# shamim-hussain/egt

Measured on AMD Instinct MI355X. Metric: graphs/sec EGT fwd+bwd, ZINC-500K padded N=64, higher is better.
Workload: dtype f32; 1 GPU; zinc500k_n64: attention-block stack (h,e,mask)->(h',e') x Ly, fwd+bwd + param grads; scope=stack, graphs_per_gpu=128, global_batch=128, N=64, Dh=64, De=64, H=8, d=8, Ly=10, parallelism=dp1, grad_allreduce_bytes=740480, backend=none (single process), flat_grad_adopted=True, flat_grad_bound=True, collective_in_graph=False

## Files before the change

### egt_amd/_lib.py

```python
from __future__ import annotations

import ctypes as C
import os

_HERE = os.path.dirname(os.path.abspath(__file__))
LIB_PATH = os.environ.get("EGT_AMD_LIB") or os.path.join(_HERE, "lib", "libegt_amd.so")

ABI_VERSION = 4
EGT_OK = 0
EGT_E_NULL, EGT_E_SHAPE, EGT_E_DTYPE, EGT_E_FLAGS, EGT_E_HIP, EGT_E_WORKSPACE, EGT_E_RCCL = -1, -2, -3, -4, -5, -6, -7
EGT_F32 = 0
EGT_BF16 = 1
F_EDGE_INPUT, F_GATE_INPUT, F_ATTN_MASK, F_SCALE_DEGREE = 0x001, 0x002, 0x004, 0x008
F_SCALER_LINEAR, F_TRAINING, F_CLIP = 0x010, 0x020, 0x040
ATTN_WS_SHARED = 0x1
EP_LAYERNORM, EP_GATES = 0x1, 0x2
ACT_NONE, ACT_LRELU, ACT_RELU, ACT_ELU = 0, 1, 2, 3
BF_GATE, BF_ATTN_MASK, BF_TRAINING, BF_CLIP, BF_NO_EDGE_LN, BF_SEED_DEVICE = 0x1, 0x2, 0x4, 0x8, 0x10, 0x20
BF_STATIC_EDGE = 0x40


class AttnDesc(C.Structure):
    _fields_ = [("B", C.c_int32), ("N", C.c_int32), ("H", C.c_int32), ("d", C.c_int32),
                ("dtype", C.c_int32), ("flags", C.c_uint32),
                ("clip_lo", C.c_float), ("clip_hi", C.c_float),
                ("random_mask_prob", C.c_float), ("attn_dropout", C.c_float),
                ("num_virtual_nodes", C.c_int32), ("reserved", C.c_int32),
                ("seed", C.c_uint64)]


class EdgeDesc(C.Structure):
    _fields_ = [("rows", C.c_int64), ("De", C.c_int32), ("H", C.c_int32),
                ("dtype", C.c_int32), ("flags", C.c_uint32), ("act", C.c_int32),
                ("act_alpha", C.c_float), ("ln_eps", C.c_float), ("reserved", C.c_int32)]


class BlockDesc(C.Structure):
    _fields_ = [("B", C.c_int32), ("N", C.c_int32), ("H", C.c_int32), ("d", C.c_int32),
                ("De", C.c_int32), ("dtype", C.c_int32), ("flags", C.c_uint32),
                ("clip_lo", C.c_float), ("clip_hi", C.c_float),
                ("random_mask_prob", C.c_float), ("ln_eps", C.c_float),
                ("reserved", C.c_int32), ("seed", C.c_uint64), ("seed_device", C.c_void_p)]


class FfnDesc(C.Structure):
    _fields_ = [("rows", C.c_int64), ("width", C.c_int32), ("dtype", C.c_int32),
                ("activation", C.c_int32), ("ln_eps", C.c_float), ("matmul", C.c_int32), ("flags", C.c_int32)]


MM_F32, MM_BF16X3, MM_BF16 = 0, 1, 2
FFN_WS_PREPARED = 1


FFN_PARAM_FIELDS = ("norm_gamma", "norm_beta", "lr1_kernel", "lr1_bias", "lr2_kernel", "lr2_bias")


class FfnParams(C.Structure):
    _fields_ = [(n, C.c_void_p) for n in FFN_PARAM_FIELDS]


BLOCK_PARAM_FIELDS = (
    "norm_edge_gamma", "norm_edge_beta",
    "attention_gates_kernel", "attention_gates_bias",
    "dense_edge_b_kernel", "dense_edge_b_bias",
    "norm_mha_gamma", "norm_mha_beta",
    "dense_qkv_kernel", "dense_qkv_bias",
    "dense_mha_kernel", "dense_mha_bias",
    "dense_edge_r_kernel", "dense_edge_r_bias",
)


class BlockParams(C.Structure):
    _fields_ = [(n, C.c_void_p) for n in BLOCK_PARAM_FIELDS]


class EmbedDesc(C.Structure):
    _fields_ = [("B", C.c_int32), ("N", C.c_int32), ("De", C.c_int32), ("upto_hop", C.c_int32),
                ("clip_hops", C.c_int32), ("num_edge_features", C.c_int32), ("dtype", C.c_int32),
                ("num_float_features", C.c_int32), ("mask_value", C.c_float), ("reserved", C.c_int32)]


EH_LAYERNORM = 0x1


class HeadDesc(C.Structure):
    _fields_ = [("B", C.c_int32), ("N", C.c_int32), ("De", C.c_int32), ("M0", C.c_int32), ("M1", C.c_int32),
                ("C", C.c_int32), ("dtype", C.c_int32), ("activation", C.c_int32), ("flags", C.c_int32),
                ("ln_eps", C.c_float), ("reserved", C.c_int32)]


HEAD_PARAM_FIELDS = ("edge_norm_final_gamma", "edge_norm_final_beta", "mlp_out_dist_targ_0_kernel",
                     "mlp_out_dist_targ_0_bias", "mlp_out_dist_targ_1_kernel", "mlp_out_dist_targ_1_bias",
                     "distance_target_kernel", "distance_target_bias")


class HeadParams(C.Structure):
    _fields_ = [(n, C.c_void_p) for n in HEAD_PARAM_FIELDS]


class EGTLibraryError(RuntimeError):
    pass


_lib = None

_VP = C.c_void_p
_PROTOS = {
    "egt_last_error_string": (C.c_char_p, []),
    "egt_abi_version": (C.c_int, []),
    "egt_attn_fwd": (C.c_int, [C.POINTER(AttnDesc)] + [_VP] * 12),
    "egt_attn_bwd_workspace_bytes": (C.c_size_t, [C.POINTER(AttnDesc)]),
    "egt_attn_bwd": (C.c_int, [C.POINTER(AttnDesc)] + [_VP] * 16),
    "egt_attn_mfma_supported": (C.c_int, [C.POINTER(AttnDesc), C.c_int]),
    "egt_attn_mfma_fwd_workspace_bytes": (C.c_size_t, [C.POINTER(AttnDesc)]),
    "egt_attn_mfma_workspace_bytes": (C.c_size_t, [C.POINTER(AttnDesc)]),
    "egt_attn_mfma_fwd": (C.c_int, [C.POINTER(AttnDesc)] + [_VP] * 11),
    "egt_attn_mfma_bwd": (C.c_int, [C.POINTER(AttnDesc)] + [_VP] * 15),
    "egt_mask_sample": (C.c_int, [C.c_int, C.c_uint64, C.c_float, C.c_int32, C.c_int32,
                                  C.c_int32, _VP, _VP]),
    "egt_seed_advance": (C.c_int, [_VP, C.c_int32, C.c_uint64, _VP]),
    "egt_edge_proj_fwd": (C.c_int, [C.POINTER(EdgeDesc)] + [_VP] * 10),
    "egt_edge_proj_bwd_workspace_bytes": (C.c_size_t, [C.POINTER(EdgeDesc)]),
    "egt_edge_proj_bwd": (C.c_int, [C.POINTER(EdgeDesc)] + [_VP] * 17),
    "egt_edge_proj_bwd_acc": (C.c_int, [C.POINTER(EdgeDesc)] + [_VP] * 18),
    "egt_edge_update_fwd": (C.c_int, [C.POINTER(EdgeDesc)] + [_VP] * 6),
    "egt_edge_update_bwd_workspace_bytes": (C.c_size_t, [C.POINTER(EdgeDesc)]),
    "egt_edge_update_bwd": (C.c_int, [C.POINTER(EdgeDesc)] + [_VP] * 8),
    "egt_node_mask_from_features": (C.c_int, [_VP, C.c_int32, C.c_int32, C.c_int32, _VP, _VP]),
    "egt_node_mask_from_float_features": (C.c_int, [_VP, C.c_int32, C.c_int32, C.c_int32, C.c_float, C.c_int32, _VP, _VP]),
    "egt_constrained_edge_mask": (C.c_int, [_VP, C.c_int32, C.c_int32, C.c_int32, C.c_int32, _VP, _VP]),
    "egt_edge_embed_supported": (C.c_int, [C.POINTER(EmbedDesc)]),
    "egt_edge_embed_hops_bytes": (C.c_size_t, [C.POINTER(EmbedDesc)]),
    "egt_edge_embed_workspace_bytes": (C.c_size_t, [C.POINTER(EmbedDesc)]),
    "egt_edge_embed_fwd": (C.c_int, [C.POINTER(EmbedDesc)] + [_VP] * 9),
    "egt_edge_embed_bwd": (C.c_int, [C.POINTER(EmbedDesc)] + [_VP] * 8),
    "egt_distance_target": (C.c_int, [_VP, C.c_int32, C.c_int32, C.c_int32, _VP, _VP]),
    "egt_edge_head_supported": (C.c_int, [C.POINTER(HeadDesc)]),
    "egt_edge_head_workspace_bytes": (C.c_size_t, [C.POINTER(HeadDesc)]),
    "egt_edge_head_fwd": (C.c_int, [C.POINTER(HeadDesc), C.POINTER(HeadParams)] + [_VP] * 5),
    "egt_edge_head_bwd": (C.c_int, [C.POINTER(HeadDesc), C.POINTER(HeadParams)] + [_VP] * 4
                          + [C.POINTER(HeadParams)] + [_VP] * 2),
    "egt_dp_unique_id": (C.c_int, [_VP]),
    "egt_dp_init": (C.c_int, [_VP, C.c_int32, C.c_int32]),
    "egt_dp_allreduce": (C.c_int, [_VP, C.c_size_t, C.c_int32, _VP]),
    "egt_dp_world": (C.c_int, []),
    "egt_dp_rank": (C.c_int, []),
    "egt_dp_finalize": (C.c_int, []),
    "egt_prof_enable": (C.c_int, [C.c_int]),
    "egt_prof_filter": (C.c_int, [C.c_char_p]),
    "egt_prof_stride": (C.c_int, [C.c_int]),
    "egt_prof_read": (C.c_int, [C.c_char_p, C.POINTER(C.c_int64), C.POINTER(C.c_double)]),
    "egt_prof_names": (C.c_int, [C.c_char_p, C.c_size_t]),
    "egt_prof_collect_graph": (C.c_int, [C.c_int]),
    "egt_prof_forget_graphs": (C.c_int, []),
    "egt_block_supported": (C.c_int, [C.POINTER(BlockDesc)]),
    "egt_block_bwd_kernel": (C.c_char_p, [C.POINTER(BlockDesc)]),
    "egt_block_launch_form": (C.c_char_p, [C.POINTER(BlockDesc)]),
    "egt_block_saved_bytes": (C.c_size_t, [C.POINTER(BlockDesc)]),
    "egt_block_workspace_bytes": (C.c_size_t, [C.POINTER(BlockDesc)]),
    "egt_block_fwd": (C.c_int, [C.POINTER(BlockDesc), C.POINTER(BlockParams)] + [_VP] * 10),
    "egt_block_bwd": (C.c_int, [C.POINTER(BlockDesc), C.POINTER(BlockParams)] + [_VP] * 10
                      + [C.POINTER(BlockParams)] + [_VP] * 2),
    "egt_stack_saved_bytes": (C.c_size_t, [C.POINTER(BlockDesc), C.c_int32]),
    "egt_stack_workspace_bytes": (C.c_size_t, [C.POINTER(BlockDesc), C.c_int32]),
    "egt_stack_fwd": (C.c_int, [C.POINTER(BlockDesc), C.c_int32, C.POINTER(BlockParams)] + [_VP] * 9),
    "egt_stack_bwd": (C.c_int, [C.POINTER(BlockDesc), C.c_int32, C.POINTER(BlockParams)] + [_VP] * 9
                      + [C.POINTER(BlockParams)] + [_VP] * 2),
    "egt_pair_supported": (C.c_int, [C.POINTER(BlockDesc)]),
    "egt_pair_workspace_bytes": (C.c_size_t, [C.POINTER(BlockDesc)]),
    "egt_pair_fwd": (C.c_int, [C.POINTER(BlockDesc), C.POINTER(BlockParams)] + [_VP] * 8),
    "egt_pair_bwd": (C.c_int, [C.POINTER(BlockDesc), C.POINTER(BlockParams)] + [_VP] * 9
                     + [C.POINTER(BlockParams)] + [_VP] * 2),
    "egt_ffn_supported": (C.c_int, [C.POINTER(FfnDesc)]),
    "egt_ffn_workspace_bytes": (C.c_size_t, [C.POINTER(FfnDesc)]),
    "egt_ffn_fwd": (C.c_int, [C.POINTER(FfnDesc), C.POINTER(FfnParams)] + [_VP] * 4),
    "egt_ffn_bwd": (C.c_int, [C.POINTER(FfnDesc), C.POINTER(FfnParams)] + [_VP] * 3
                    + [C.POINTER(FfnParams)] + [_VP] * 2),
}


def load():
    global _lib
    if _lib is not None:
        return _lib
    if not os.path.exists(LIB_PATH):
        raise EGTLibraryError(
            f"{LIB_PATH} not found: build the HIP extension first "
            "(python -c 'import __graft_entry__ as g; g.build()' or python egt_amd/build.py)")
    lib = C.CDLL(LIB_PATH)
    for name, (res, args) in _PROTOS.items():
        fn = getattr(lib, name)
        fn.restype, fn.argtypes = res, args
    if lib.egt_abi_version() != ABI_VERSION:
        raise EGTLibraryError("ABI version mismatch")
    _lib = lib
    return lib


_EXC = {EGT_E_NULL: ValueError, EGT_E_SHAPE: AssertionError, EGT_E_DTYPE: TypeError,
        EGT_E_FLAGS: ValueError, EGT_E_HIP: RuntimeError, EGT_E_WORKSPACE: RuntimeError, EGT_E_RCCL: RuntimeError}


def check(rc: int):
    if rc == EGT_OK:
        return
    msg = load().egt_last_error_string().decode(errors="replace")
    raise _EXC.get(rc, RuntimeError)(f"egt_amd: {msg} (code {rc})")


def ptr(t):
    return None if t is None else C.c_void_p(t.data_ptr())


def current_stream():
    import torch
    return C.c_void_p(torch.cuda.current_stream().cuda_stream)
```

### egt_amd/csrc/egt_block.hip

```cpp
#include "egt_common.h"

#include <stdio.h>
#include <stdlib.h>
#include <string.h>
#include <vector>

#include "egt_block.h"
#include "egt_tile.h"

#include "egt_block_dev.h"
#include "egt_dma.h"

#include "egt_block_fwd.h"
#include "egt_block_bwd.h"



struct EgtBlockEnv {
  bool no_narrow_fwd, no_narrow_bwd;
  int bwd_mm;
  int bwd_tl, fwd_rows;
  int nrw_fwd_waves, nrw_bwd_waves, nrw_fwd_half;
};
static bool env_flag_raw(const char* name) {
  const char* v = getenv(name);
  return v && v[0] && v[0] != '0';
}
static int env_int(const char* name, int unset) {
  const char* v = getenv(name);
  return v ? atoi(v) : unset;
}
static const EgtBlockEnv& block_env() {
  static const EgtBlockEnv e = [] {
    EgtBlockEnv v{};
    v.no_narrow_fwd = env_flag_raw("EGT_NO_NARROW_FWD") || env_flag_raw("EGT_NO_NARROW");
    v.no_narrow_bwd = env_flag_raw("EGT_NO_NARROW_BWD") || env_flag_raw("EGT_NO_NARROW");
    const char* mm = getenv("EGT_BWD_MATMUL");
    v.bwd_mm = (mm && !strcmp(mm, "bf16x3")) ? EGT_MM_BF16X3 : EGT_MM_F32;
    v.bwd_tl = env_int("EGT_BWD_TL", 0);
    v.fwd_rows = env_int("EGT_FWD_ROWS", 0);
    v.nrw_fwd_waves = env_int("EGT_NRW_FWD_WAVES", 0);
    v.nrw_bwd_waves = env_int("EGT_NRW_BWD_WAVES", 0);
    v.nrw_fwd_half = env_int("EGT_NRW_FWD_HALF", -1);
    return v;
  }();
  return e;
}
int egt_device_cus() {
  static const int n = [] {
    int dev = 0, cu = 256;
    if (hipGetDevice(&dev) == hipSuccess) (void)hipDeviceGetAttribute(&cu, hipDeviceAttributeMultiprocessorCount, dev);
    return cu > 0 ? cu : 256;
  }();
  return n;
}

static int block_check(const egt_block_desc* d, bool report) {
#define BAD(code, ...) do { if (report) egt_set_error(__VA_ARGS__); return (code); } while (0)
  if (!d) BAD(EGT_E_NULL, "desc is NULL");
  if (d->dtype != EGT_F32 && d->dtype != EGT_BF16) BAD(EGT_E_DTYPE, "dtype must be EGT_F32 or EGT_BF16 (got %d)", d->dtype);
  if (d->B <= 0 || d->N <= 0) BAD(EGT_E_SHAPE, "B and N must be positive");
  if (d->H != BH) BAD(EGT_E_SHAPE, "fused block is built for num_heads=8 (got %d)", d->H);
  if (d->d < 1 || d->d > 8) BAD(EGT_E_SHAPE, "fused block covers per-head dim <= 8 (got %d)", d->d);
  switch (d->De) {
    case 8: case 16: case 32: case 48: case 64: break;
    default: BAD(EGT_E_SHAPE, "fused block covers edge_width in {8,16,32,48,64} (got %d)", d->De);
  }
  if ((size_t)d->B * d->N * d->N * d->H > 0xFFFFFFFFull) BAD(EGT_E_SHAPE, "B*N*N*H exceeds the 32-bit RNG counter");
  if ((d->flags & EGT_BF_SEED_DEVICE) && !d->seed_device) BAD(EGT_E_NULL, "EGT_BF_SEED_DEVICE set but seed_device is NULL");
  if (d->flags & EGT_BF_STATIC_EDGE) {
    if (!(d->flags & EGT_BF_NO_EDGE_LN)) BAD(EGT_E_FLAGS, "EGT_BF_STATIC_EDGE is only valid together with EGT_BF_NO_EDGE_LN");
    if (d->flags & EGT_BF_ATTN_MASK) BAD(EGT_E_FLAGS, "EGT_BF_STATIC_EDGE does not take EGT_BF_ATTN_MASK");
    if (d->De != 8) BAD(EGT_E_SHAPE, "EGT_BF_STATIC_EDGE covers edge_width 8 (got %d)", d->De);
    if (block_env().no_narrow_fwd || block_env().no_narrow_bwd) BAD(EGT_E_FLAGS, "EGT_BF_STATIC_EDGE needs the De = 8 pair kernels (EGT_NO_NARROW* is set)");
  }
  return EGT_OK;
#undef BAD
}

extern "C" int egt_block_supported(const egt_block_desc* d) { return block_check(d, false) == EGT_OK; }

static size_t al(size_t x) { return (x + 63) & ~(size_t)63; }

enum class FwdKernel { narrow, r4, tile };
enum class BwdKernel { narrow, v4r, v5, v4 };
static const char* const g_bwd_kernel_name[] = {"k_narrow_bwd", "k_block_bwd_v4r", "k_block_bwd_v5", "k_block_bwd_v4"};
constexpr int V4R_RR = 2;

struct BlockPlan {
  bool ml;
  bool full;
  FwdKernel fwd;
  EgtLaunch fl;
  int fwd_nw;
  bool fwd_half;
  bool kvl;
  bool epi_ok;
  int RGF;
  BwdKernel bwd;
  EgtLaunch bl;
  int bwd_nw;
  int mm;
  int TL, NLR, nwg_bwd, EP;
  size_t v_att, stats, qkvp, pw_sv, wfrag_sv, saved_total;
  size_t dvp, dqp, dkvp, dqp_sz, dkvp_sz, common_total;
  size_t pw, epart, spart, sbo, wpart, ered, dqkv, dhbuf, layer_total;
};

template <int DE>
static BlockPlan plan_for(const egt_block_desc* d, bool ml) {
  using GG = Geo<DE>;
  const EgtBlockEnv& E = block_env();
  const int B = d->B, N = d->N, cus = egt_device_cus();
  const int groups = (N + BWD_TL - 1) / BWD_TL;
  BlockPlan P{};
  P.ml = ml;
  P.full = (N % 16) == 0;

  int tg = 2 * cus / B;
  {
    const int cap = B * ((N + 3) / 4) <= cus ? (N + 3) / 4 : (N + 7) / 8;
    if (tg > cap) tg = cap;
  }

  P.RGF = tg > groups ? (((N + tg - 1) / tg + 3) / 4) * 4 : 16;
  if (E.fwd_rows >= 4 && E.fwd_rows <= 16) P.RGF = E.fwd_rows;
  const size_t lds_tiles = (size_t)8 * GG::TILE_FLOATS * 4;
  const size_t lds_kv = ((size_t)N * KV_LD + 16 * QS_LD + N) * 4;
  P.kvl = lds_tiles + lds_kv <= 80 * 1024 - 512;
  const size_t lds_r4 = (size_t)16 * GG::TILE_FLOATS * 4 + lds_kv;
  const size_t lds_r8 = (size_t)32 * GG::TILE_FLOATS * 4 + ((size_t)N * KV_LD + 32 * QS_LD + N) * 4;
  const bool r4 = lds_r4 <= 80 * 1024 - 512, r8 = !r4 && lds_r8 <= 156 * 1024;
  if (DE == 8 && !ml && !E.no_narrow_fwd) {
    const int grid16 = B * groups;
    P.fwd = FwdKernel::narrow;
    P.fwd_nw = E.nrw_fwd_waves == 8 || (E.nrw_fwd_waves != 4 && grid16 <= cus && N >= 64) ? 8 : 4;
    P.fwd_half = P.fwd_nw == 8 && (E.nrw_fwd_half == 1 || (E.nrw_fwd_half != 0 && 2 * grid16 <= cus));
    P.fl = {P.fwd_half ? B * ((N + 7) / 8) : grid16, 64 * P.fwd_nw, egt_narrow_fwd_lds(P.fwd_nw)};
  } else if (DE <= 16 && !ml && (r4 || r8)) {
    P.fwd = FwdKernel::r4;
    P.fwd_nw = r4 ? 4 : 8;
    P.fl = {B * ((N + 4 * P.fwd_nw - 1) / (4 * P.fwd_nw)), 64 * P.fwd_nw, r4 ? lds_r4 : lds_r8};
  } else {
    P.fwd = FwdKernel::tile;
    P.fl = {B * ((N + P.RGF - 1) / P.RGF), 256, lds_tiles + (P.kvl ? lds_kv : 0)};
  }
  P.epi_ok = P.fwd != FwdKernel::tile || P.kvl;

  if (E.bwd_tl >= 4 && E.bwd_tl <= BWD_TL) P.TL = E.bwd_tl;
  else if (DE != 8) {
    const int g = tg > groups ? tg : groups;
    P.TL = (N + g - 1) / g;
  } else if (B * groups <= cus) {
    P.TL = BWD_TL;
    if (N > 8)
      for (int tl = 8; tl < BWD_TL; ++tl)
        if (B * ((N + tl - 1) / tl) <= cus) { P.TL = tl; break; }
  } else P.TL = (N + groups - 1) / groups;
  P.NLR = (N + P.TL - 1) / P.TL;
  P.nwg_bwd = B * P.NLR;
  P.EP = GG::EP;
  if (DE == 8 && !ml && !E.no_narrow_bwd) {
    P.bwd = BwdKernel::narrow;
    P.bwd_nw = E.nrw_bwd_waves == 8 || (E.nrw_bwd_waves != 4 && P.nwg_bwd <= cus && N >= 64) ? 8 : 4;
    P.bl = {P.nwg_bwd, 64 * P.bwd_nw, egt_narrow_bwd_lds(P.bwd_nw)};
  } else if (DE <= 16 && !ml) {
    constexpr int PWR = V4R_RR * (2 * GG::TILE_FLOATS + 256 + 192);
    P.bwd = BwdKernel::v4r;
    P.bl = {P.nwg_bwd, 256,
            ((size_t)(4 * PWR > BWD_PRO_WS ? 4 * PWR : BWD_PRO_WS) + (size_t)BWD_TL * QD_LD + 3 * GG::TILES * 256 + 3 * 2048 + 4) * 4};
  } else if (DE >= 32 && !ml && d->dtype != EGT_BF16) {
    P.bwd = BwdKernel::v5;
    P.mm = E.bwd_mm;
    P.bl = {P.nwg_bwd, 256, ((size_t)V5_AREA(DE) + (size_t)BWD_TL * QD_LD + 3 * ((GG::TILES + 1) / 2) * 512 + 4) * 4};
  } else {
    constexpr int PW = 3 * GG::TILE_FLOATS + 256 + 192;
    P.bwd = BwdKernel::v4;
    P.bl = {P.nwg_bwd, 256,
            ((size_t)(4 * PW > BWD_PRO_WS ? 4 * PW : BWD_PRO_WS) + (size_t)BWD_TL * QD_LD + 3 * ((GG::TILES + 1) / 2) * 512) * 4};
  }

  const size_t rows = (size_t)B * N;
  const int Dh = d->d * d->H;
  size_t o = 0;
  P.v_att = o; o += al(rows * Dh);
  P.stats = o; o += al(rows * BH * 4);
  P.qkvp = o; o += al(rows * QKVP);
  P.pw_sv = o; o += al((size_t)GG::DEP * 16 + 16);
  P.wfrag_sv = o; o += al(Dh <= 64 ? WFRAG_FLOATS : 0);
  P.saved_total = o;
  o = 0;
  P.dvp = o; o += al(rows * 64);
  P.dqp_sz = al(rows * 64 * (size_t)groups);
  P.dkvp_sz = al((size_t)P.nwg_bwd * N * 128);
  P.dqp = o; o += 2 * P.dqp_sz;
  P.dkvp = o; o += 2 * P.dkvp_sz;
  P.common_total = o;
  o = 0;
  P.pw = o; o += al((size_t)GG::DEP * 16 + 16);
  P.epart = o; o += al((size_t)P.nwg_bwd * P.EP);
  {
    const int node_wg = B * ((N + NODE_RC - 1) / NODE_RC);
    const size_t nmax = (size_t)(P.nwg_bwd > node_wg ? P.nwg_bwd : node_wg);
    P.spart = o; o += al(nmax * (5 * Dh));
    P.sbo = o; o += al(nmax * Dh);
  }
  P.wpart = o; o += al((size_t)egt_node_wgrad_chunks((int)rows, 1) * (Dh * 3 * Dh + Dh * Dh));
  P.ered = o; o += al(P.EP);
  P.dqkv = o; o += al(rows * 3 * Dh);
  P.dhbuf = o; o += al(rows * Dh);
  P.layer_total = o;
  return P;
}

#define DISPATCH_BDE(De, CALL)                        \
  switch (De) {                                       \
    case 8: { constexpr int DE = 8; CALL; } break;    \
    case 16: { constexpr int DE = 16; CALL; } break;  \
    case 32: { constexpr int DE = 32; CALL; } break;  \
    case 48: { constexpr int DE = 48; CALL; } break;  \
    default: { constexpr int DE = 64; CALL; } break;  \
  }

static BlockPlan plan_block(const egt_block_desc* d, bool ml) {
  DISPATCH_BDE(d->De, return plan_for<DE>(d, ml));
}

static bool host_rand_mask(const egt_block_desc* d, const uint8_t* rm) {
  return rm && (d->flags & EGT_BF_TRAINING) && d->random_mask_prob > 0.0f;
}
static bool mask_tensor(const egt_block_desc* d, const uint8_t* rm) {
  return (d->flags & EGT_BF_ATTN_MASK) || host_rand_mask(d, rm);
}

static void bind_ws(const BlockPlan& P, BlockArgs& a, float* wc, float* wl, int parity = 0) {
  a.dvp = wc + P.dvp; a.dqp = wc + P.dqp + parity * P.dqp_sz; a.dkvp = wc + P.dkvp + parity * P.dkvp_sz;
  a.epart = wl + P.epart; a.spart = wl + P.spart; a.sbo = wl + P.sbo; a.wpart = wl + P.wpart;
  a.spart_n = a.sbo_n = a.B * ((a.N + NODE_RC - 1) / NODE_RC);
  a.ered = wl + P.ered; a.dqkv_sv = wl + P.dqkv;
  a.TL = P.TL; a.NLR = P.NLR; a.NQP = 1;
  a.xcd = 1;
}

extern "C" const char* egt_block_bwd_kernel(const egt_block_desc* d) {
  if (block_check(d, false)) return nullptr;
  return g_bwd_kernel_name[(int)plan_block(d, mask_tensor(d, nullptr)).bwd];
}

extern "C" const char* egt_block_launch_form(const egt_block_desc* d) {
  if (block_check(d, false)) return nullptr;
  const BlockPlan P = plan_block(d, mask_tensor(d, nullptr));
  static const char* const fwd_name[] = {"k_narrow_fwd", "k_block_fwd_r4", "k_block_fwd"};
  static thread_local char buf[128];
  snprintf(buf, sizeof buf, "fwd=%s/%dw%s bwd=%s/%dw/tl%d", fwd_name[(int)P.fwd], P.fwd == FwdKernel::tile ? 4 : P.fwd_nw,
           P.fwd_half ? "/half" : "", g_bwd_kernel_name[(int)P.bwd], P.bwd == BwdKernel::narrow ? P.bwd_nw : 4, P.TL);
  return buf;
}

static int check_table(const egt_block_params* t, uint32_t flags, const char* what, int layer = -1) {
  const void* const* tp = reinterpret_cast<const void* const*>(t);
  for (int i = 0; i < 14; ++i) {
    if (tp[i] || (!(flags & EGT_BF_GATE) && (i == 2 || i == 3))) continue;
    if ((flags & EGT_BF_STATIC_EDGE) && (i < 2 || i >= 12)) continue;
    if (layer < 0) EGT_FAIL(EGT_E_NULL, "%s #%d is NULL", what, i);
    EGT_FAIL(EGT_E_NULL, "layer %d %s #%d is NULL", layer, what, i);
  }
  return EGT_OK;
}

static void fill_block(const egt_block_desc* d, const egt_block_params* p, BlockArgs& a) {
  a = BlockArgs{};
  a.B = d->B; a.N = d->N; a.De = d->De; a.DK = d->d; a.Dh = d->d * d->H;
  a.flags = d->flags;
  a.bf16 = d->dtype == EGT_BF16;
  a.clip_lo = d->clip_lo; a.clip_hi = d->clip_hi;
  a.scale = 1.0f / sqrtf((float)d->d);
  a.ln_eps = d->ln_eps;
  a.rm_thr = egt_threshold24(d->random_mask_prob);
  a.s0 = (uint32_t)(d->seed & 0xFFFFFFFFull);
  a.s1 = (uint32_t)(d->seed >> 32);
  a.sd = (d->flags & EGT_BF_SEED_DEVICE) ? (const uint32_t*)d->seed_device : nullptr;
  a.ne_g = (const float*)p->norm_edge_gamma; a.ne_b = (const float*)p->norm_edge_beta;
  a.Wg = (const float*)p->attention_gates_kernel; a.bg = (const float*)p->attention_gates_bias;
  a.We = (const float*)p->dense_edge_b_kernel; a.be = (const float*)p->dense_edge_b_bias;
  a.nm_g = (const float*)p->norm_mha_gamma; a.nm_b = (const float*)p->norm_mha_beta;
  a.Wqkv = (const float*)p->dense_qkv_kernel; a.bqkv = (const float*)p->dense_qkv_bias;
  a.Wo = (const float*)p->dense_mha_kernel; a.bo = (const float*)p->dense_mha_bias;
  a.Wr = (const float*)p->dense_edge_r_kernel; a.br = (const float*)p->dense_edge_r_bias;
  if (d->flags & EGT_BF_STATIC_EDGE) a.ne_g = a.ne_b = a.Wr = a.br = nullptr;
}

static void bind_grads(BlockArgs& a, const egt_block_params* g) {
  a.g_ne_g = (float*)g->norm_edge_gamma; a.g_ne_b = (float*)g->norm_edge_beta;
  a.g_Wg = (float*)g->attention_gates_kernel; a.g_bg = (float*)g->attention_gates_bias;
  a.g_We = (float*)g->dense_edge_b_kernel; a.g_be = (float*)g->dense_edge_b_bias;
  a.g_nm_g = (float*)g->norm_mha_gamma; a.g_nm_b = (float*)g->norm_mha_beta;
  a.g_Wqkv = (float*)g->dense_qkv_kernel; a.g_bqkv = (float*)g->dense_qkv_bias;
  a.g_Wo = (float*)g->dense_mha_kernel; a.g_bo = (float*)g->dense_mha_bias;
  a.g_Wr = (float*)g->dense_edge_r_kernel; a.g_br = (float*)g->dense_edge_r_bias;
  if (a.flags & EGT_BF_STATIC_EDGE) a.g_ne_g = a.g_ne_b = a.g_Wr = a.g_br = nullptr;
}

static void bind_common(const egt_block_desc* d, BlockArgs& a, const uint8_t* km, const void* M, const uint8_t* rm) {
  a.km = km;
  a.M = (d->flags & EGT_BF_ATTN_MASK) ? (const float*)M : nullptr;
  a.rm = nullptr; a.rng_rm = 0;
  if ((d->flags & EGT_BF_TRAINING) && d->random_mask_prob > 0.0f) {
    if (rm) a.rm = rm; else a.rng_rm = 1;
  }
  a.prep = 1;
}

static bool node_fused_ok(const BlockArgs& a) {
  return a.Dh == BH * a.DK && a.DK >= 1 && a.DK <= 8 && a.wfrag != nullptr;
}

template <int DE, bool BF>
static void launch_r4(BlockArgs& a, const BlockPlan& P, hipStream_t st) {
  if (P.fwd_nw == 4) {
    if (P.full) egt_launch_planned<k_block_fwd_r4<DE, true, 4, BF>>("k_block_fwd", P.fl, st, a);
    else egt_launch_planned<k_block_fwd_r4<DE, false, 4, BF>>("k_block_fwd", P.fl, st, a);
  } else {
    if (P.full) egt_launch_planned<k_block_fwd_r4<DE, true, 8, BF>>("k_block_fwd", P.fl, st, a);
    else egt_launch_planned<k_block_fwd_r4<DE, false, 8, BF>>("k_block_fwd", P.fl, st, a);
  }
}
template <int DE, bool BF>
static void launch_tile_fwd(BlockArgs& a, const BlockPlan& P, hipStream_t st) {
  if (!P.kvl) {
    if (P.ml) egt_launch_planned<k_block_fwd<DE, false, true, false, BF>>("k_block_fwd", P.fl, st, a);
    else egt_launch_planned<k_block_fwd<DE, false, false, false, BF>>("k_block_fwd", P.fl, st, a);
  } else if (P.ml) egt_launch_planned<k_block_fwd<DE, true, true, false, BF>>("k_block_fwd", P.fl, st, a);
  else if (P.full) egt_launch_planned<k_block_fwd<DE, true, false, true, BF>>("k_block_fwd", P.fl, st, a);
  else egt_launch_planned<k_block_fwd<DE, true, false, false, BF>>("k_block_fwd", P.fl, st, a);
}
template <int DE>
static void launch_v5(BlockArgs& a, const BlockPlan& P, hipStream_t st) {
  if (P.mm == EGT_MM_BF16X3) {
    if (P.full) egt_launch_planned<k_block_bwd_v5<DE, EGT_MM_BF16X3, false>>("k_block_bwd", P.bl, st, a);
    else egt_launch_planned<k_block_bwd_v5<DE, EGT_MM_BF16X3, true>>("k_block_bwd", P.bl, st, a);
  } else {
    if (P.full) egt_launch_planned<k_block_bwd_v5<DE, EGT_MM_F32, false>>("k_block_bwd", P.bl, st, a);
    else egt_launch_planned<k_block_bwd_v5<DE, EGT_MM_F32, true>>("k_block_bwd", P.bl, st, a);
  }
}
template <int DE, bool BF>
static void launch_v4(BlockArgs& a, const BlockPlan& P, hipStream_t st) {
  if (P.ml) {
    if (P.full) egt_launch_planned<k_block_bwd_v4<DE, true, BF, false>>("k_block_bwd", P.bl, st, a);
    else egt_launch_planned<k_block_bwd_v4<DE, true, BF, true>>("k_block_bwd", P.bl, st, a);
  } else {
    if (P.full) egt_launch_planned<k_block_bwd_v4<DE, false, BF, false>>("k_block_bwd", P.bl, st, a);
    else egt_launch_planned<k_block_bwd_v4<DE, false, BF, true>>("k_block_bwd", P.bl, st, a);
  }
}

template <int DE>
static int launch_fwd(BlockArgs& a, const BlockPlan& P, hipStream_t st, bool skip_pre) {
  if (!skip_pre) egt_node_launch_pre(a, st);
  if (!(P.epi_ok && node_fused_ok(a))) a.epi = 0;
  a.guard = 0;
  a.RGF = P.RGF;
  switch (P.fwd) {
    case FwdKernel::narrow: egt_narrow_launch_fwd(a, P.fwd_nw, P.fwd_half, P.fl, st); break;
    case FwdKernel::r4:
      if constexpr (DE <= 16) { if (a.bf16) launch_r4<DE, true>(a, P, st); else launch_r4<DE, false>(a, P, st); }
      break;
    case FwdKernel::tile: if (a.bf16) launch_tile_fwd<DE, true>(a, P, st); else launch_tile_fwd<DE, false>(a, P, st); break;
  }
  if (a.epi == 0) egt_node_launch_post(a, st);
  return a.epi;
}

template <int DE>
static void launch_bwd(BlockArgs& a, const BlockPlan& P, hipStream_t st, bool top, BlockArgs* below, BlockArgs* above, bool fuse) {
  static_assert(DE % 16 == 0 || DE == 8, "edge widths of the pair kernels");
  const bool pro = fuse;
  a.pro = 0;
  if (pro) {
    a.pro = top ? 1 : 2;
    a.sbo_n = P.nwg_bwd;
    if (!top) {
      a.up_h = above->h; a.up_nm_g = above->nm_g; a.up_Wqkv = above->Wqkv; a.up_wfrag = above->wfrag; a.up_dh_out = above->dh_out;
      a.up_dqp = above->dqp; a.up_dkvp = above->dkvp; a.up_dqkv_sv = above->dqkv_sv; a.up_spart = above->spart;
      above->spart_n = P.nwg_bwd;
    }
    if (a.prep) egt_node_launch_prep(&a, 1, st);
  } else if (top) {
    egt_node_launch_bwd(a, &a, false, st);
  }
  a.NQP = (a.N + 15) / 16;
  a.guard = 0;
  switch (P.bwd) {
    case BwdKernel::narrow: egt_narrow_launch_bwd(a, P.bwd_nw, P.bl, st); break;
    case BwdKernel::v4r:
      if constexpr (DE <= 16) {
        if (a.bf16) egt_launch_planned<k_block_bwd_v4r<DE, true, V4R_RR>>("k_block_bwd", P.bl, st, a);
        else egt_launch_planned<k_block_bwd_v4r<DE, false, V4R_RR>>("k_block_bwd", P.bl, st, a);
      }
      break;
    case BwdKernel::v5:
      if constexpr (DE >= 32) launch_v5<DE>(a, P, st);
      break;
    case BwdKernel::v4: if (a.bf16) launch_v4<DE, true>(a, P, st); else launch_v4<DE, false>(a, P, st); break;
  }
  if (!pro) egt_node_launch_bwd(a, below, true, st);
  else if (!below) egt_node_launch_bwd(a, nullptr, true, st);
}

static uint64_t layer_seed(uint64_t seed, int l) { return seed ^ (0x9E3779B97F4A7C15ull * (uint64_t)(l + 1)); }

struct StackLayout {
  size_t h_act, e_act, blk, saved_total;
  size_t ws_total;
  size_t h_sz, e_sz;
};

static int stack_flags_check(const egt_block_desc* d, bool report) {
  if (d && (d->flags & EGT_BF_STATIC_EDGE)) {
    if (report) egt_set_error("egt_stack_* does not take EGT_BF_STATIC_EDGE (use egt_block_fwd / egt_block_bwd per layer)");
    return EGT_E_FLAGS;
  }
  return EGT_OK;
}

static StackLayout stack_layout(const egt_block_desc* d, const BlockPlan& P, int layers) {
  StackLayout S{};
  S.h_sz = al((size_t)d->B * d->N * d->d * d->H);
  S.e_sz = al((size_t)d->B * d->N * d->N * d->De / (d->dtype == EGT_BF16 ? 2 : 1));
  size_t o = 0;
  S.h_act = o; o += S.h_sz * (size_t)(layers > 1 ? layers - 1 : 0);
  S.e_act = o; o += S.e_sz * (size_t)(layers > 1 ? layers - 1 : 0);
  S.blk = o; o += P.saved_total * (size_t)layers;
  S.saved_total = o;
  S.ws_total = P.common_total + P.layer_total * (size_t)layers;
  return S;
}

static size_t chain_bytes(const egt_block_desc* d, int layers, bool stack, bool ws) {
  if ((stack && stack_flags_check(d, false)) || block_check(d, false) || layers < 1) return 0;
  const StackLayout S = stack_layout(d, plan_block(d, mask_tensor(d, nullptr)), layers);
  return (ws ? S.ws_total : S.saved_total) * sizeof(float);
}
extern "C" size_t egt_block_saved_bytes(const egt_block_desc* d) { return chain_bytes(d, 1, false, false); }
extern "C" size_t egt_block_workspace_bytes(const egt_block_desc* d) { return chain_bytes(d, 1, false, true); }
extern "C" size_t egt_stack_saved_bytes(const egt_block_desc* d, int32_t layers) { return chain_bytes(d, layers, true, false); }
extern "C" size_t egt_stack_workspace_bytes(const egt_block_desc* d, int32_t layers) { return chain_bytes(d, layers, true, true); }

static void bind_layer(const StackLayout& S, const BlockPlan& P, int l, BlockArgs& a, float* saved, float* ws) {
  float* bs = saved + S.blk + P.saved_total * (size_t)l;
  a.v_att = bs + P.v_att; a.stats = bs + P.stats; a.qkvp = bs + P.qkvp;
  bind_ws(P, a, ws, ws + P.common_total + P.layer_total * (size_t)l, l & 1);
  a.pw = bs + P.pw_sv;
  a.wfrag = a.Dh <= 64 ? bs + P.wfrag_sv : nullptr;
}

struct ChainCall {
  const egt_block_desc* d;
  int layers;
  bool stack, bwd;
  const egt_block_params *params, *grads;
  const void *h, *e;
  const uint8_t* km;
  const void* M;
  const uint8_t* rm;
  float *saved, *ws;
};

static int check_call(const ChainCall& c, bool ptrs_ok, const char* names, bool alias) {
  const egt_block_desc* d = c.d;
  int rc;
  if (c.stack) {
    if ((rc = stack_flags_check(d, true))) return rc;
    if (c.layers < 1) EGT_FAIL(EGT_E_SHAPE, "layers must be >= 1");
    if (c.bwd && c.layers > 64) EGT_FAIL(EGT_E_SHAPE, "at most 64 layers per stack call");
    if (!ptrs_ok) EGT_FAIL(EGT_E_NULL, "params/%s is NULL", names);
    if ((rc = block_check(d, true))) return rc;
  } else {
    if ((rc = block_check(d, true))) return rc;
    if (!c.params) EGT_FAIL(EGT_E_NULL, "params is NULL");
    if ((rc = check_table(c.params, d->flags, "block parameter"))) return rc;
    if (!ptrs_ok) EGT_FAIL(EGT_E_NULL, "%s is NULL", names);
  }
  if ((d->flags & EGT_BF_ATTN_MASK) && !c.M) EGT_FAIL(EGT_E_NULL, "ATTN_MASK set but attn_mask is NULL");
  if ((d->flags & EGT_BF_STATIC_EDGE) && host_rand_mask(d, c.rm))
    EGT_FAIL(EGT_E_FLAGS, "EGT_BF_STATIC_EDGE takes the in-kernel random mask only (rand_mask must be NULL)");
  if (c.layers > 64) EGT_FAIL(EGT_E_SHAPE, "at most 64 layers per stack call");
  if (alias) EGT_FAIL(EGT_E_FLAGS, "d_h must not alias d_h_out (d_e may alias d_e_out)");
  return EGT_OK;
}

static int bind_chain(const ChainCall& c, const BlockPlan& P, BlockArgs* as) {
  const StackLayout S = stack_layout(c.d, P, c.layers);
  for (int i = 0; i < c.layers; ++i) {
    const int l = c.bwd ? c.layers - 1 - i : i;
    int rc = c.stack ? check_table(c.params + l, c.d->flags, "block parameter") : EGT_OK;
    if (!rc && c.bwd) rc = check_table(c.grads + l, c.d->flags, "gradient pointer", c.stack ? l : -1);
    if (rc) return rc;
    egt_block_desc dl = *c.d;
    if (c.stack) dl.seed = layer_seed(c.d->seed, l);
    BlockArgs& a = as[l];
    fill_block(&dl, c.params + l, a);
    a.h = l == 0 ? (const float*)c.h : c.saved + S.h_act + S.h_sz * (size_t)(l - 1);
    a.e = l == 0 ? (const float*)c.e : c.saved + S.e_act + S.e_sz * (size_t)(l - 1);
    bind_common(&dl, a, c.km, c.M, c.rm);
    bind_layer(S, P, l, a, c.saved, c.ws);
    if (c.bwd) bind_grads(a, c.grads + l);
  }
  return EGT_OK;
}

extern "C" int egt_block_fwd(const egt_block_desc* desc, const egt_block_params* params,
                             const void* h, const void* e, const uint8_t* key_mask,
                             const void* attn_mask, const uint8_t* rand_mask, void* h_out,
                             void* e_out, void* saved, void* workspace, void* stream) {
  const bool se = desc && (desc->flags & EGT_BF_STATIC_EDGE);
  const ChainCall c{desc, 1, false, false, params, nullptr, h, e, key_mask, attn_mask, rand_mask, (float*)saved, (float*)workspace};
  int rc = check_call(c, h && e && h_out && (e_out || se) && saved && workspace, "h/e/h_out/e_out/saved/workspace", false);
  if (rc) return rc;
  const BlockPlan P = plan_block(desc, mask_tensor(desc, rand_mask));
  BlockArgs a;
  if ((rc = bind_chain(c, P, &a))) return rc;
  a.h_out = (float*)h_out; a.e_out = se ? nullptr : (float*)e_out;
  a.epi = 1;
  DISPATCH_BDE(desc->De, launch_fwd<DE>(a, P, (hipStream_t)stream, false));
  EGT_HIP_LAUNCH_CHECK("egt_block_fwd");
  return EGT_OK;
}

extern "C" int egt_block_bwd(const egt_block_desc* desc, const egt_block_params* params,
                             const void* h, const void* e, const uint8_t* key_mask,
                             const void* attn_mask, const uint8_t* rand_mask, const void* saved,
                             const void* d_h_out, const void* d_e_out, void* d_h, void* d_e,
                             const egt_block_params* grads, void* workspace, void* stream) {
  const bool se = desc && (desc->flags & EGT_BF_STATIC_EDGE);
  const ChainCall c{desc, 1, false, true, params, grads, h, e, key_mask, attn_mask, rand_mask, (float*)saved, (float*)workspace};
  int rc = check_call(c, h && e && saved && d_h_out && (d_e_out || se) && d_h && d_e && grads && workspace,
                      "h/e/saved/d_h_out/d_e_out/d_h/d_e/grads/workspace", d_h == d_h_out);
  if (rc) return rc;
  const BlockPlan P = plan_block(desc, mask_tensor(desc, rand_mask));
  BlockArgs a;
  if ((rc = bind_chain(c, P, &a))) return rc;
  a.prep = 0;
  a.dh_out = (const float*)d_h_out; a.de_out = (const float*)d_e_out;
  a.dh = (float*)d_h; a.de = (float*)d_e;
  DISPATCH_BDE(desc->De, launch_bwd<DE>(a, P, (hipStream_t)stream, true, nullptr, nullptr, node_fused_ok(a)));
  egt_node_launch_wgrads(&a, 1, (hipStream_t)stream);
  egt_node_launch_reduce(&a, 1, P.nwg_bwd, P.EP, (hipStream_t)stream);
  EGT_HIP_LAUNCH_CHECK("egt_block_bwd");
  return EGT_OK;
}


extern "C" int egt_stack_fwd(const egt_block_desc* desc, int32_t layers, const egt_block_params* params,
                             const void* h, const void* e, const uint8_t* key_mask,
                             const void* attn_mask, void* h_out, void* e_out, void* saved,
                             void* workspace, void* stream) {
  const ChainCall c{desc, layers, true, false, params, nullptr, h, e, key_mask, attn_mask, nullptr, (float*)saved, (float*)workspace};
  int rc = check_call(c, params && h && e && h_out && e_out && saved && workspace, "h/e/h_out/e_out/saved/workspace", false);
  if (rc) return rc;
  const BlockPlan P = plan_block(desc, mask_tensor(desc, nullptr));
  BlockArgs as[64];
  if ((rc = bind_chain(c, P, as))) return rc;
  for (int l = 0; l < layers; ++l) {
    as[l].h_out = l == layers - 1 ? (float*)h_out : const_cast<float*>(as[l + 1].h);
    as[l].e_out = l == layers - 1 ? (float*)e_out : const_cast<float*>(as[l + 1].e);
  }
  for (int l = 0; l < layers; ++l) as[l].prep = 0;
  int prev_epi = 0;
  if (egt_node_launch_pre_stack(as, layers, (hipStream_t)stream)) prev_epi = 2;
  else egt_node_launch_prep(as, layers, (hipStream_t)stream);
  for (int l = 0; l < layers; ++l) {
    BlockArgs& a = as[l];
    a.epi = 1;
    if (l + 1 < layers) {
      const BlockArgs& nx = as[l + 1];
      a.epi = 2;
      a.nx_nm_g = nx.nm_g; a.nx_nm_b = nx.nm_b; a.nx_Wqkv = nx.Wqkv; a.nx_wfrag = nx.wfrag; a.nx_bqkv = nx.bqkv;
      a.nx_qkvp = nx.qkvp;
    }
    DISPATCH_BDE(desc->De, prev_epi = launch_fwd<DE>(a, P, (hipStream_t)stream, prev_epi == 2));
  }
  EGT_HIP_LAUNCH_CHECK("egt_stack_fwd");
  return EGT_OK;
}

extern "C" int egt_stack_bwd(const egt_block_desc* desc, int32_t layers, const egt_block_params* params,
                             const void* h, const void* e, const uint8_t* key_mask,
                             const void* attn_mask, const void* saved, const void* d_h_out,
                             const void* d_e_out, void* d_h, void* d_e,
                             const egt_block_params* grads, void* workspace, void* stream) {
  const ChainCall c{desc, layers, true, true, params, grads, h, e, key_mask, attn_mask, nullptr, (float*)saved, (float*)workspace};
  int rc = check_call(c, params && grads && h && e && saved && d_h_out && d_e_out && d_h && d_e && workspace,
                      "grads/h/e/saved/d_h_out/d_e_out/d_h/d_e/workspace", d_h == d_h_out);
  if (rc) return rc;
  const BlockPlan P = plan_block(desc, mask_tensor(desc, nullptr));
  BlockArgs as[64];
  if ((rc = bind_chain(c, P, as))) return rc;
  for (int l = 0; l < layers; ++l) {
    BlockArgs& a = as[l];
    auto dhbuf = [&](int ll) { return (float*)workspace + P.common_total + P.layer_total * (size_t)ll + P.dhbuf; };
    a.dh_out = l == layers - 1 ? (const float*)d_h_out : (const float*)dhbuf(l + 1);
    a.de_out = l == layers - 1 ? (const float*)d_e_out : (const float*)d_e;
    a.dh = l == 0 ? (float*)d_h : dhbuf(l);
    a.de = (float*)d_e;
  }
  bool fuse = true;
  for (int l = 0; l < layers; ++l) fuse = fuse && node_fused_ok(as[l]);
  for (int l = layers - 1; l >= 0; --l) {
    as[l].prep = 0;
    DISPATCH_BDE(desc->De, launch_bwd<DE>(as[l], P, (hipStream_t)stream, l == layers - 1, l > 0 ? &as[l - 1] : nullptr,
                                          l + 1 < layers ? &as[l + 1] : nullptr, fuse));
  }
  egt_node_launch_wgrads(as, layers, (hipStream_t)stream);
  egt_node_launch_reduce(as, layers, P.nwg_bwd, P.EP, (hipStream_t)stream);
  EGT_HIP_LAUNCH_CHECK("egt_stack_bwd");
  return EGT_OK;
}
```

### egt_amd/csrc/egt_block_bwd.h

```cpp
#pragma once
#ifndef EGT_NT_BWD_E
#define EGT_NT_BWD_E true
#endif
#ifndef EGT_NT_BWD_DY
#define EGT_NT_BWD_DY false
#endif
#ifndef EGT_NT_BWD_ST
#define EGT_NT_BWD_ST false
#endif

template <int DE, bool ML, bool BF, bool RAG>
__global__ void __launch_bounds__(256, 2) k_block_bwd_v4(BlockArgs a) {
  seed_from_device(a);
  using G = Geo<DE>;
  typedef typename EdgeT<BF>::type ET;
  const ET* e_in = reinterpret_cast<const ET*>(a.e);
  ET* e_o = reinterpret_cast<ET*>(a.e_out);
  const ET* dey_in = reinterpret_cast<const ET*>(a.de_out);
  ET* dex_o = reinterpret_cast<ET*>(a.de);
  (void)e_in; (void)e_o; (void)dey_in; (void)dex_o;
  extern __shared__ __attribute__((aligned(16))) float sm[];
  const int lane = threadIdx.x & 63, wave = threadIdx.x >> 6;
  const int p = lane & 15, q = lane >> 4;
  const int N = a.N, TL = a.TL;
  const int wg = a.xcd ? egt_xcd_remap(blockIdx.x, gridDim.x) : (int)blockIdx.x;
  const int b = wg / a.NLR, lr = wg % a.NLR;
  const int l_begin = lr * TL, l_end = min(N, l_begin + TL), nl = l_end - l_begin;
  const bool gated = (a.flags & EGT_BF_GATE) != 0;
  const bool clip = (a.flags & EGT_BF_CLIP) != 0;
  constexpr int PW = 3 * G::TILE_FLOATS + 256 + 192;
  constexpr int WSLAB = G::TILES * 256;
  float* et = sm + wave * PW;
  float* dt0 = et + G::TILE_FLOATS;
  float* sc1 = dt0 + 2 * G::TILE_FLOATS;
  float* sc2 = sc1 + 256;
  constexpr int AREA = 4 * PW > BWD_PRO_WS ? 4 * PW : BWD_PRO_WS;
  float* qd = sm + AREA;
  float* wsA = qd + TL * QD_LD;
  float* wsB = wsA + WSLAB;
  float* wsD = wsB + WSLAB;
  bwd_stage_rows<256, 3>(a, qd, b, l_begin, nl);
  if (a.pro) {
    __syncthreads();
    bwd_node_prologue<DE>(a, sm, qd, b, l_begin, wg);
  }
  for (int i = threadIdx.x; i < G::TILES * 256; i += 256) {
    const int t = i >> 8, ln = (i >> 2) & 63, u = i & 3, pp = ln & 15, qq = ln >> 4;
    const int c = 16 * t + 4 * qq + u;
    wsA[i] = a.pw[c * 16 + pp];
    const int hd = 2 * (pp >> 2) + (pp & 1);
    wsB[i] = ((pp & 2) == 0 && c < DE) ? a.Wr[hd * DE + c] : 0.f;
    wsD[i] = a.pw[(16 * t + pp) * 16 + 4 * qq + u];
  }
  float c2r[4];
#pragma unroll
  for (int r = 0; r < 4; ++r) c2r[r] = a.pw[G::DEP * 16 + 4 * q + r];

  v4f accT[G::TILES], accR[G::TILES];
#pragma unroll
  for (int t = 0; t < G::TILES; ++t) { accT[t] = (v4f){0.f, 0.f, 0.f, 0.f}; accR[t] = (v4f){0.f, 0.f, 0.f, 0.f}; }
  float ssum[4] = {0.f, 0.f, 0.f, 0.f};
  __syncthreads();

  const int ntile = RAG ? (N + 15) / 16 : N / 16;
  for (int mt = wave; mt < ntile; mt += 4) {
    const int m0 = mt * 16, m = m0 + p;
    const int kv = RAG ? min(16, N - m0) : 16;
    const bool kvalid = RAG ? (m < N) : true;
    float Kf[16], Vf[16], dKa[16], dVa[16];
    const size_t rowm = (size_t)b * N + (kvalid ? m : N - 1);
    {
      const float4* kp = reinterpret_cast<const float4*>(a.qkvp + rowm * QKVP + 64 + q * 16);
      const float4* vp = reinterpret_cast<const float4*>(a.qkvp + rowm * QKVP + 128 + q * 16);
#pragma unroll
      for (int i = 0; i < 4; ++i) {
        const float4 kv = kp[i], vv = vp[i];
        Kf[4*i] = kv.x; Kf[4*i+1] = kv.y; Kf[4*i+2] = kv.z; Kf[4*i+3] = kv.w;
        Vf[4*i] = vv.x; Vf[4*i+1] = vv.y; Vf[4*i+2] = vv.z; Vf[4*i+3] = vv.w;
      }
#pragma unroll
      for (int i = 0; i < 16; ++i) { dKa[i] = 0.f; dVa[i] = 0.f; }
    }
    const float kadd = (a.km && a.km[rowm] == 0) ? -EGT_NEG : 0.0f;

    TileRegs<DE> te, td;
    for (int l = l_begin; l < l_end; ++l) {
      const int li = l - l_begin;
      const size_t rowl = (size_t)b * N + l;
      const size_t pair0 = rowl * N + m0;
      float* dt = dt0 + (li & 1) * G::TILE_FLOATS;
      MaskRegs mr{make_float2(1.f, 1.f), 0};
      mask_gload<ML>(a, mr, pair0 + (kvalid ? p : 0), q);
      lds_sync();
      if (li > 0)
        tile_from_lds<DE>(dt0 + ((li - 1) & 1) * G::TILE_FLOATS, dex_o + (pair0 - (size_t)N) * DE, lane, kv);
      const size_t lp0 = (a.guard & 16) ? (size_t)wave * 16 : pair0;
      tile_gload<DE>(td, dey_in + lp0 * DE, lane, kv);
      tile_gload<DE>(te, e_in + lp0 * DE, lane, kv);
      tile_lds_put<DE>(et, te, lane, kv);
      tile_lds_put<DE>(dt, td, lane, kv);
      lds_sync();
      SCHED_FENCE();
      float rstd;
      v4f acc = {c2r[0], c2r[1], c2r[2], c2r[3]};
      {
        float4 x[G::TILES];
#pragma unroll
        for (int t = 0; t < G::TILES; ++t) x[t] = frag_read<DE>(et, p, q, t);
        rstd = ln_frags<DE>(x, q, a.ln_eps, (a.flags & EGT_BF_NO_EDGE_LN) == 0);
#pragma unroll
        for (int t = 0; t < G::TILES; ++t) {
          frag_write<DE>(et, p, q, t, x[t]);
          const float4 w = *reinterpret_cast<const float4*>(wsA + (t * 64 + lane) * 4);
          acc = MFMA(w.x, x[t].x, acc);
          acc = MFMA(w.y, x[t].y, acc);
          acc = MFMA(w.z, x[t].z, acc);
          acc = MFMA(w.w, x[t].w, acc);
        }
      }
      SCHED_FENCE();
      v4f dhx = {0.f, 0.f, 0.f, 0.f};
      if (!(a.guard & 8))
#pragma unroll
      for (int t = 0; t < G::TILES; ++t) {
        const float4 dyv = frag_read<DE>(dt, p, q, t);
        const float4 w = *reinterpret_cast<const float4*>(wsB + (t * 64 + lane) * 4);
        dhx = MFMA(w.x, dyv.x, dhx);
        dhx = MFMA(w.y, dyv.y, dhx);
        dhx = MFMA(w.z, dyv.z, dhx);
        dhx = MFMA(w.w, dyv.w, dhx);
      }
      SCHED_FENCE();
      float dge[4], hh[2], dA[2], at[2];
      {
        const float* qr = qd + li * QD_LD;
        float dots[2], dAd[2];
        {
          const float4* qp = reinterpret_cast<const float4*>(qr + q * 16);
          const float4* dp = reinterpret_cast<const float4*>(qr + 64 + q * 16);
          float d0 = 0.f, d1 = 0.f, e0 = 0.f, e1 = 0.f;
#pragma unroll
          for (int i = 0; i < 4; ++i) {
            const float4 u = qp[i], v = dp[i];
            d0 = fmaf(u.x, Kf[4*i], d0);   d1 = fmaf(u.y, Kf[4*i+1], d1);
            d0 = fmaf(u.z, Kf[4*i+2], d0); d1 = fmaf(u.w, Kf[4*i+3], d1);
            e0 = fmaf(v.x, Vf[4*i], e0);   e1 = fmaf(v.y, Vf[4*i+1], e1);
            e0 = fmaf(v.z, Vf[4*i+2], e0); e1 = fmaf(v.w, Vf[4*i+3], e1);
          }
          dots[0] = d0; dots[1] = d1; dAd[0] = e0; dAd[1] = e1;
        }
        const float4* sp = reinterpret_cast<const float4*>(qr + 128 + q * 8);
        const float4 s0 = sp[0], s1 = sp[1];
        const float st[8] = {s0.x, s0.y, s0.z, 0.f, s1.x, s1.y, s1.z, 0.f};
        float xl[2], gl[2], inr[2];
#pragma unroll
        for (int j = 0; j < 2; ++j) {
          const float araw = dots[j] * a.scale;
          float ah = araw;
          inr[j] = 1.0f;
          if (clip) {
            inr[j] = (araw >= a.clip_lo && araw <= a.clip_hi) ? 1.0f : 0.0f;
            ah = fminf(fmaxf(araw, a.clip_lo), a.clip_hi);
          }
          hh[j] = ah + acc[2 * j + 1];
          xl[j] = hh[j];
          gl[j] = acc[2 * j];
        }
        apply_masks<ML>(a, kadd, mr, (pair0 + p) * BH, q, xl, gl);
        if (RAG && !kvalid) { xl[0] = xl[1] = -3.0e38f; gl[0] = gl[1] = -3.0e38f; }
#pragma unroll
        for (int j = 0; j < 2; ++j) {
          const float S = __expf(xl[j] - st[4 * j]) * st[4 * j + 1];
          const float g = gated ? egt_sigmoid(gl[j]) : 1.0f;
          const float dS = dAd[j] * g;
          const float dGl = gated ? dAd[j] * S * g * (1.0f - g) : 0.f;
          const float dH = S * (dS - st[4 * j + 2]) + dhx[j];
          dA[j] = dH * inr[j] * a.scale;
          at[j] = S * g;
          dge[2 * j] = dGl;
          dge[2 * j + 1] = dH;
        }
      }
#pragma unroll
      for (int r = 0; r < 4; ++r) ssum[r] += dge[r];
      *reinterpret_cast<float4*>(sc1 + p * 16 + 4 * q) = make_float4(dge[0], dge[1], dge[2], dge[3]);
      *reinterpret_cast<float2*>(sc2 + p * 12 + 2 * q) = make_float2(hh[0], hh[1]);
      if (q == 0) sc2[p * 12 + 8] = 1.0f;
      lds_sync();
      SCHED_FENCE();
      if (!(a.guard & 4)) {
        const float* qr = qd + li * QD_LD;
        const float4* qp = reinterpret_cast<const float4*>(qr + q * 16);
        const float4* dp = reinterpret_cast<const float4*>(qr + 64 + q * 16);
        float dq[16];
#pragma unroll
        for (int i = 0; i < 4; ++i) {
          const float4 u = qp[i], v = dp[i];
          dKa[4*i]   = fmaf(dA[0], u.x, dKa[4*i]);   dKa[4*i+1] = fmaf(dA[1], u.y, dKa[4*i+1]);
          dKa[4*i+2] = fmaf(dA[0], u.z, dKa[4*i+2]); dKa[4*i+3] = fmaf(dA[1], u.w, dKa[4*i+3]);
          dVa[4*i]   = fmaf(at[0], v.x, dVa[4*i]);   dVa[4*i+1] = fmaf(at[1], v.y, dVa[4*i+1]);
          dVa[4*i+2] = fmaf(at[0], v.z, dVa[4*i+2]); dVa[4*i+3] = fmaf(at[1], v.w, dVa[4*i+3]);
        }
#pragma unroll
        for (int k = 0; k < 8; ++k) { dq[2 * k] = dA[0] * Kf[2 * k]; dq[2 * k + 1] = dA[1] * Kf[2 * k + 1]; }
        a.dqp[(((size_t)b * ntile + mt) * N + l) * 64 + lane] = reduce16_keep_own(dq, p);
      }
      SCHED_FENCE();
      if (!(a.guard & 1)) {
        float bT[4], bR[4];
#pragma unroll
        for (int s = 0; s < 4; ++s) {
          bT[s] = sc1[(q + 4 * s) * 16 + p];
          bR[s] = (p < 9) ? sc2[(q + 4 * s) * 12 + p] : 0.f;
        }
#pragma unroll
        for (int t = 0; t < G::TILES; ++t)
#pragma unroll
          for (int s = 0; s < 4; ++s) {
            accT[t] = MFMA(elem_read<DE>(et, q + 4 * s, 16 * t + p), bT[s], accT[t]);
            accR[t] = MFMA(elem_read<DE>(dt, q + 4 * s, 16 * t + p), bR[s], accR[t]);
          }
      }
      lds_sync();
      SCHED_FENCE();
      if (!(a.guard & 2)) {
        float4 dxh[G::TILES];
        float m1 = 0.f, m2 = 0.f;
#pragma unroll
        for (int t = 0; t < G::TILES; ++t) {
          const float4 w = *reinterpret_cast<const float4*>(wsD + (t * 64 + lane) * 4);
          const float4 xh = frag_read<DE>(et, p, q, t);
          v4f d = {0.f, 0.f, 0.f, 0.f};
          d = MFMA(w.x, dge[0], d);
          d = MFMA(w.y, dge[1], d);
          d = MFMA(w.z, dge[2], d);
          d = MFMA(w.w, dge[3], d);
          dxh[t] = make_float4(d[0], d[1], d[2], d[3]);
          m1 += (d[0] + d[1]) + (d[2] + d[3]);
          m2 = fmaf(d[0], xh.x, m2); m2 = fmaf(d[1], xh.y, m2);
          m2 = fmaf(d[2], xh.z, m2); m2 = fmaf(d[3], xh.w, m2);
        }
        m1 = sum_over_q(m1) * (1.0f / DE);
        m2 = sum_over_q(m2) * (1.0f / DE);
        if (a.flags & EGT_BF_NO_EDGE_LN) { m1 = 0.f; m2 = 0.f; }
        lds_sync();
#pragma unroll
        for (int t = 0; t < G::TILES; ++t) {
          const float4 dyv = frag_read<DE>(dt, p, q, t);
          const float4 xh = frag_read<DE>(et, p, q, t);
          float4 o;
          o.x = dyv.x + rstd * (dxh[t].x - m1 - xh.x * m2);
          o.y = dyv.y + rstd * (dxh[t].y - m1 - xh.y * m2);
          o.z = dyv.z + rstd * (dxh[t].z - m1 - xh.z * m2);
          o.w = dyv.w + rstd * (dxh[t].w - m1 - xh.w * m2);
          frag_write<DE>(dt, p, q, t, o);
        }
      }
      SCHED_FENCE();
    }
    {
      lds_sync();
      tile_from_lds<DE>(dt0 + ((nl - 1) & 1) * G::TILE_FLOATS,
                        dex_o + (((size_t)b * N + l_end - 1) * N + m0) * DE, lane, kv);
    }
    float4* ko = reinterpret_cast<float4*>(a.dkvp + (((((size_t)b * a.NLR + lr) * N + m) * 2 + 0) * 4 + q) * 16);
    float4* vo = reinterpret_cast<float4*>(a.dkvp + (((((size_t)b * a.NLR + lr) * N + m) * 2 + 1) * 4 + q) * 16);
    if (kvalid) {
#pragma unroll
      for (int i = 0; i < 4; ++i) {
        ko[i] = make_float4(dKa[4*i], dKa[4*i+1], dKa[4*i+2], dKa[4*i+3]);
        vo[i] = make_float4(dVa[4*i], dVa[4*i+1], dVa[4*i+2], dVa[4*i+3]);
      }
    }
  }
#pragma unroll
  for (int r = 0; r < 4; ++r) ssum[r] = row_sum16(ssum[r]);
  __syncthreads();
  float* ep = sm + wave * G::EP;
#pragma unroll
  for (int t = 0; t < G::TILES; ++t)
#pragma unroll
    for (int r = 0; r < 4; ++r) {
      ep[(16 * t + 4 * q + r) * 16 + p] = accT[t][r];
      ep[G::DEP * 16 + 16 + (16 * t + 4 * q + r) * 16 + p] = accR[t][r];
    }
  if (p == 0) {
#pragma unroll
    for (int r = 0; r < 4; ++r) ep[G::DEP * 16 + 4 * q + r] = ssum[r];
  }
  __syncthreads();
  float* out = a.epart + (size_t)wg * G::EP;
  for (int i = threadIdx.x; i < G::EP; i += 256)
    out[i] = (sm[i] + sm[G::EP + i]) + (sm[2 * G::EP + i] + sm[3 * G::EP + i]);
}

#define V5_AREA(DE_) ((4 * (3 * Geo<DE_>::TILE_FLOATS + 448) > 4 * Geo<DE_>::TILE_FLOATS + BWD_PRO_WS) \
                          ? 4 * (3 * Geo<DE_>::TILE_FLOATS + 448) : 4 * Geo<DE_>::TILE_FLOATS + BWD_PRO_WS)
template <int DE, int MM, bool RAG>
__global__ void __launch_bounds__(256, 2) k_block_bwd_v5(BlockArgs a) {
  seed_from_device(a);
  constexpr bool SPLIT = MM == EGT_MM_BF16X3;
  constexpr int NS = (Geo<DE>::TILES + 1) / 2;
  (void)SPLIT; (void)NS;
  using G = Geo<DE>;
  const float* e_in = a.e;
  const float* dey_in = a.de_out;
  float* dex_o = a.de;
  extern __shared__ __attribute__((aligned(16))) float sm[];
  const int lane = threadIdx.x & 63, wave = __builtin_amdgcn_readfirstlane(threadIdx.x >> 6);
  const int p = lane & 15, q = lane >> 4;
  const int N = a.N, TL = a.TL;
  const int wg = a.xcd ? egt_xcd_remap(blockIdx.x, gridDim.x) : (int)blockIdx.x;
  const int b = wg / a.NLR, lr = wg % a.NLR;
  const int l_begin = lr * TL, l_end = min(N, l_begin + TL), nl = l_end - l_begin;
  const bool gated = (a.flags & EGT_BF_GATE) != 0;
  const bool clip = (a.flags & EGT_BF_CLIP) != 0;
  constexpr int PW = 3 * G::TILE_FLOATS + 256 + 192;
  constexpr int WSLAB = (MM != 0 && NS * 512 > G::TILES * 256) ? NS * 512 : G::TILES * 256;
  constexpr int PW2 = 2 * G::TILE_FLOATS + 256 + 192;
  float* et0 = sm + wave * G::TILE_FLOATS;
  float* et1 = sm + 4 * G::TILE_FLOATS + wave * PW2;
  const int estr = __builtin_amdgcn_readfirstlane((int)(et1 - et0));
  float* dt = et1 + G::TILE_FLOATS;
  float* sc1 = dt + G::TILE_FLOATS;
  float* sc2 = sc1 + 256;
  constexpr int AREA = V5_AREA(DE);
  static_assert(4 * PW == 4 * G::TILE_FLOATS + 4 * PW2 && AREA >= 4 * PW && AREA >= 4 * G::TILE_FLOATS + BWD_PRO_WS, "tile area");
  float* pro_ws = sm + 4 * G::TILE_FLOATS;
  float* qd = sm + AREA;
  float* wsA = qd + TL * QD_LD;
  float* wsB = wsA + WSLAB;
  float* wsD = wsB + WSLAB;
  volatile int* pflag = reinterpret_cast<volatile int*>(wsD + WSLAB);
  if (threadIdx.x < 4) pflag[threadIdx.x] = 0;
  const unsigned et_lds = __builtin_amdgcn_readfirstlane((unsigned)(size_t)et0);
  const unsigned off0 = dma_lane_offset<DE>(lane);
  const int ntile = RAG ? (N + 15) / 16 : N / 16;
  const bool balance = RAG && ntile >= 3 && (ntile & 3) != 0;
  const int T_ = ntile * nl;
  const int t0 = balance ? (wave * T_) >> 2 : 0, t1 = balance ? ((wave + 1) * T_) >> 2 : 0;
  const bool have = balance ? t1 > t0 : wave < ntile;
  const int mt_first = balance ? t0 / nl : wave, mt_last = balance ? (t1 - 1) / nl : ntile - 1, mt_step = balance ? 1 : 4;
  const int r0_first = balance ? t0 - mt_first * nl : 0;
  float Kf[16], Vf[16];
  int kmv = 1;
#define V5_TILE_START(MT_, ROW_)                                                                                    \
  do {                                                                                                              \
    const int m0_ = (MT_) * 16, kv_ = RAG ? min(16, N - m0_) : 16;                                                  \
    if (RAG && kv_ < 16) tile_dma_ragged<DE>(et_lds, e_in + (((size_t)b * N + l_begin + (ROW_)) * N + m0_) * DE, lane, kv_); \
    else tile_dma<DE, EGT_NT_BWD_E>(et_lds, e_in + (((size_t)b * N + l_begin + (ROW_)) * N + m0_) * DE, off0);      \
    const size_t rowm_ = (size_t)b * N + (RAG ? min(m0_ + p, N - 1) : m0_ + p);                                     \
    const float4* kp_ = reinterpret_cast<const float4*>(a.qkvp + rowm_ * QKVP + 64 + q * 16);                       \
    const float4* vp_ = reinterpret_cast<const float4*>(a.qkvp + rowm_ * QKVP + 128 + q * 16);                      \
    _Pragma("unroll") for (int i = 0; i < 4; ++i) {                                                                 \
      const float4 kv4 = kp_[i], vv4 = vp_[i];                                                                      \
      Kf[4*i] = kv4.x; Kf[4*i+1] = kv4.y; Kf[4*i+2] = kv4.z; Kf[4*i+3] = kv4.w;                                     \
      Vf[4*i] = vv4.x; Vf[4*i+1] = vv4.y; Vf[4*i+2] = vv4.z; Vf[4*i+3] = vv4.w;                                     \
    }                                                                                                               \
    kmv = a.km ? (int)a.km[rowm_] : 1;                                                                              \
  } while (0)
  if (have) V5_TILE_START(mt_first, r0_first);
  BwdProRegs proR;
  {
    float4 sv[3];
#pragma unroll
    for (int u = 0; u < 3; ++u) {
      const int i = threadIdx.x + 256 * u, r = i / 40, f = i % 40;
      const bool ok = i < nl * 40 && !(a.pro && f >= 16 && f < 32);
      const size_t rowl = (size_t)b * N + l_begin + (ok ? r : 0);
      const float* src = f < 16 ? a.qkvp + rowl * QKVP + f * 4
                       : f < 32 ? a.dvp + rowl * 64 + (f - 16) * 4
                                : a.stats + rowl * 32 + (f - 32) * 4;
      sv[u] = ok ? *reinterpret_cast<const float4*>(src) : make_float4(0.f, 0.f, 0.f, 0.f);
    }
    float sA[G::TILES], sB[G::TILES], sD[G::TILES];
    if constexpr (MM == 0) {
#pragma unroll
      for (int t = 0; t < G::TILES; ++t) {
        const int i = threadIdx.x + 256 * t, ln = (i >> 2) & 63, u = i & 3, pp = ln & 15, qq = ln >> 4;
        const int c = 16 * t + 4 * qq + u;
        const int hd = 2 * (pp >> 2) + (pp & 1);
        sA[t] = a.pw[c * 16 + pp];
        sB[t] = ((pp & 2) == 0 && c < DE) ? a.Wr[hd * DE + c] : 0.f;
        sD[t] = a.pw[(16 * t + pp) * 16 + 4 * qq + u];
      }
    }
    if (a.pro) bwd_node_prologue_load<DE>(a, proR, b, l_begin);
#pragma unroll
    for (int u = 0; u < 3; ++u) {
      const int i = threadIdx.x + 256 * u, r = i / 40, f = i % 40;
      if (i < nl * 40 && !(a.pro && f >= 16 && f < 32)) {
        float4 v = sv[u];
        if (f >= 32) v.y = 1.0f / v.y;
        *reinterpret_cast<float4*>(qd + r * QD_LD + f * 4) = v;
      }
    }
    if constexpr (MM == 0) {
#pragma unroll
      for (int t = 0; t < G::TILES; ++t) {
        const int i = threadIdx.x + 256 * t;
        wsA[i] = sA[t]; wsB[i] = sB[t]; wsD[i] = sD[t];
      }
    }
  }
  if (a.pro) {
    __syncthreads();
    bwd_node_prologue_finish<DE>(a, pro_ws, qd, b, l_begin, wg, proR);
  }
  if constexpr (MM != 0) {
    uint16_t* A16 = reinterpret_cast<uint16_t*>(wsA);
    uint16_t* B16 = reinterpret_cast<uint16_t*>(wsB);
    uint16_t* D16 = reinterpret_cast<uint16_t*>(wsD);
    auto parts = [](float v, uint16_t& hi, uint16_t& lo) {
      const uint32_t h = pk_bf16(v, 0.f) & 0xFFFFu;
      hi = (uint16_t)h;
      lo = (uint16_t)(pk_bf16(v - __uint_as_float(h << 16), 0.f) & 0xFFFFu);
    };
    for (int idx = threadIdx.x; idx < NS * 512; idx += 256) {
      const int i = idx & 7, ln = (idx >> 3) & 63, s_ = idx >> 9, pp = ln & 15, qq = ln >> 4, t = 2 * s_ + (i >> 2);
      const int c = 16 * t + 4 * qq + (i & 3);
      const bool in = t < G::TILES && c < DE;
      const int hd = 2 * (pp >> 2) + (pp & 1);
      uint16_t hi, lo;
      parts(in ? a.pw[c * 16 + pp] : 0.f, hi, lo);
      A16[((s_ * 2 + 0) * 64 + ln) * 8 + i] = hi; A16[((s_ * 2 + 1) * 64 + ln) * 8 + i] = lo;
      parts((in && (pp & 2) == 0) ? a.Wr[hd * DE + c] : 0.f, hi, lo);
      B16[((s_ * 2 + 0) * 64 + ln) * 8 + i] = hi; B16[((s_ * 2 + 1) * 64 + ln) * 8 + i] = lo;
    }
    for (int idx = threadIdx.x; idx < G::TILES * 256; idx += 256) {
      const int u = idx & 3, ln = (idx >> 2) & 63, t = idx >> 8, pp = ln & 15, qq = ln >> 4;
      uint16_t hi, lo;
      parts(a.pw[(16 * t + pp) * 16 + 4 * qq + u], hi, lo);
      D16[(t * 64 + ln) * 8 + u] = hi; D16[(t * 64 + ln) * 8 + 4 + u] = lo;
    }
  }
  float c2r[4];
#pragma unroll
  for (int r = 0; r < 4; ++r) c2r[r] = a.pw[G::DEP * 16 + 4 * q + r];

  v4f accT[G::TILES], accR[G::TILES];
#pragma unroll
  for (int t = 0; t < G::TILES; ++t) { accT[t] = (v4f){0.f, 0.f, 0.f, 0.f}; accR[t] = (v4f){0.f, 0.f, 0.f, 0.f}; }
  float ssum[4] = {0.f, 0.f, 0.f, 0.f};
  __syncthreads();

  for (int mt = mt_first; have && mt <= mt_last; mt += mt_step) {
    const int r0 = (balance && mt == mt_first) ? r0_first : 0;
    const int r1 = (balance && mt == mt_last) ? t1 - mt * nl : nl;
    const int m0 = mt * 16, m = m0 + p;
    const int kv = RAG ? min(16, N - m0) : 16;
    const bool kvalid = RAG ? (p < kv) : true;
    if (mt != mt_first) V5_TILE_START(mt, r0);
    float dKa[16], dVa[16];
#pragma unroll
    for (int i = 0; i < 16; ++i) { dKa[i] = 0.f; dVa[i] = 0.f; }
    asm volatile("" : "+v"(kmv));
    const float kadd = kmv == 0 ? -EGT_NEG : 0.0f;
    const int l_first = l_begin + r0, l_stop = l_begin + r1;
    for (int l = l_first; l < l_stop; ++l) {
      const int li = l - l_begin;
      const int lj = l - l_first;
      const size_t rowl = (size_t)b * N + l;
      const size_t pair0 = rowl * N + m0;
      float* et = et0 + (lj & 1) * estr;
      MaskRegs mr{make_float2(1.f, 1.f), 0};
      TileRegs<DE> td;
      tile_gload<DE, EGT_NT_BWD_DY>(td, dey_in + pair0 * DE, lane, kv);
      if (lj == 0) vm_wait<(G::NF4 + 63) / 64>(); else vm_wait<2 * ((G::NF4 + 63) / 64) + 1>();
      SCHED_FENCE();
      float rstd;
      v4f acc = {c2r[0], c2r[1], c2r[2], c2r[3]};
      {
        float4 x[G::TILES];
#pragma unroll
        for (int t = 0; t < G::TILES; ++t) x[t] = frag_read<DE>(et, p, q, t);
        rstd = ln_frags<DE>(x, q, a.ln_eps, (a.flags & EGT_BF_NO_EDGE_LN) == 0);
        if constexpr (MM != 0) {
#pragma unroll
          for (int t = 0; t < G::TILES; ++t) frag_write<DE>(et, p, q, t, x[t]);
          v4f xv[G::TILES];
          Bf8 xh[NS], xl[NS];
#pragma unroll
          for (int t = 0; t < G::TILES; ++t) xv[t] = (v4f){x[t].x, x[t].y, x[t].z, x[t].w};
          split_tiles<G::TILES, SPLIT>(xv, xh, xl);
          acc = bf_gemm<NS, SPLIT>(wsA, 0, lane, xh, xl, acc);
        } else {
#pragma unroll
        for (int t = 0; t < G::TILES; ++t) {
          frag_write<DE>(et, p, q, t, x[t]);
          const float4 w = *reinterpret_cast<const float4*>(wsA + (t * 64 + lane) * 4);
          acc = MFMA(w.x, x[t].x, acc);
          acc = MFMA(w.y, x[t].y, acc);
          acc = MFMA(w.z, x[t].z, acc);
          acc = MFMA(w.w, x[t].w, acc);
        }
        }
      }
      SCHED_FENCE();
      tile_lds_put<DE>(dt, td, lane, kv);
      lds_sync();
      if (l + 1 < l_stop) {
        if (RAG && kv < 16) tile_dma_ragged<DE>(et_lds + (unsigned)(((lj + 1) & 1) * estr * 4), e_in + (pair0 + (size_t)N) * DE, lane, kv);
        else tile_dma<DE, EGT_NT_BWD_E>(et_lds + (unsigned)(((lj + 1) & 1) * estr * 4), e_in + (pair0 + (size_t)N) * DE, off0);
      }
      SCHED_FENCE();
      v4f dhx = {0.f, 0.f, 0.f, 0.f};
      if (!(a.guard & 8)) {
      if constexpr (MM != 0) {
        v4f dv[G::TILES];
        Bf8 dh_[NS], dl_[NS];
#pragma unroll
        for (int t = 0; t < G::TILES; ++t) { const float4 d4 = frag_read<DE>(dt, p, q, t); dv[t] = (v4f){d4.x, d4.y, d4.z, d4.w}; }
        split_tiles<G::TILES, SPLIT>(dv, dh_, dl_);
        dhx = bf_gemm<NS, SPLIT>(wsB, 0, lane, dh_, dl_, dhx);
      } else {
#pragma unroll
      for (int t = 0; t < G::TILES; ++t) {
        const float4 dyv = frag_read<DE>(dt, p, q, t);
        const float4 w = *reinterpret_cast<const float4*>(wsB + (t * 64 + lane) * 4);
        dhx = MFMA(w.x, dyv.x, dhx);
        dhx = MFMA(w.y, dyv.y, dhx);
        dhx = MFMA(w.z, dyv.z, dhx);
        dhx = MFMA(w.w, dyv.w, dhx);
      }
      }
      }
      SCHED_FENCE();
      float dge[4], hh[2], dA[2], at[2];
      {
        const float* qr = qd + li * QD_LD;
        float dots[2], dAd[2];
        {
          const float4* qp = reinterpret_cast<const float4*>(qr + q * 16);
          const float4* dp = reinterpret_cast<const float4*>(qr + 64 + q * 16);
          float d0 = 0.f, d1 = 0.f, e0 = 0.f, e1 = 0.f;
#pragma unroll
          for (int i = 0; i < 4; ++i) {
            const float4 u = qp[i], v = dp[i];
            d0 = fmaf(u.x, Kf[4*i], d0);   d1 = fmaf(u.y, Kf[4*i+1], d1);
            d0 = fmaf(u.z, Kf[4*i+2], d0); d1 = fmaf(u.w, Kf[4*i+3], d1);
            e0 = fmaf(v.x, Vf[4*i], e0);   e1 = fmaf(v.y, Vf[4*i+1], e1);
            e0 = fmaf(v.z, Vf[4*i+2], e0); e1 = fmaf(v.w, Vf[4*i+3], e1);
          }
          dots[0] = d0; dots[1] = d1; dAd[0] = e0; dAd[1] = e1;
        }
        const float4* sp = reinterpret_cast<const float4*>(qr + 128 + q * 8);
        const float4 s0 = sp[0], s1 = sp[1];
        const float st[8] = {s0.x, s0.y, s0.z, 0.f, s1.x, s1.y, s1.z, 0.f};
        float xl[2], gl[2], inr[2];
#pragma unroll
        for (int j = 0; j < 2; ++j) {
          const float araw = dots[j] * a.scale;
          float ah = araw;
          inr[j] = 1.0f;
          if (clip) {
            inr[j] = (araw >= a.clip_lo && araw <= a.clip_hi) ? 1.0f : 0.0f;
            ah = fminf(fmaxf(araw, a.clip_lo), a.clip_hi);
          }
          hh[j] = ah + acc[2 * j + 1];
          xl[j] = hh[j];
          gl[j] = acc[2 * j];
        }
        apply_masks<false>(a, kadd, mr, (pair0 + p) * BH, q, xl, gl);
        if (RAG && !kvalid) { xl[0] = xl[1] = -3.0e38f; gl[0] = gl[1] = -3.0e38f; }
#pragma unroll
        for (int j = 0; j < 2; ++j) {
          const float S = __expf(xl[j] - st[4 * j]) * st[4 * j + 1];
          const float g = (gated || (RAG && !kvalid)) ? egt_sigmoid(gl[j]) : 1.0f;
          const float dS = dAd[j] * g;
          const float dGl = gated ? dAd[j] * S * g * (1.0f - g) : 0.f;
          const float dH = S * (dS - st[4 * j + 2]) + dhx[j];
          dA[j] = dH * inr[j] * a.scale;
          at[j] = S * g;
          dge[2 * j] = dGl;
          dge[2 * j + 1] = dH;
        }
      }
#pragma unroll
      for (int r = 0; r < 4; ++r) ssum[r] += dge[r];
      *reinterpret_cast<float4*>(sc1 + p * 16 + 4 * q) = make_float4(dge[0], dge[1], dge[2], dge[3]);
      *reinterpret_cast<float2*>(sc2 + p * 12 + 2 * q) = make_float2(hh[0], hh[1]);
      if (q == 0) sc2[p * 12 + 8] = 1.0f;
      lds_sync();
      SCHED_FENCE();
      if (!(a.guard & 4))
      {
        const float* qr = qd + li * QD_LD;
        const float4* qp = reinterpret_cast<const float4*>(qr + q * 16);
        const float4* dp = reinterpret_cast<const float4*>(qr + 64 + q * 16);
        float dq[16];
#pragma unroll
        for (int i = 0; i < 4; ++i) {
          const float4 u = qp[i], v = dp[i];
          dKa[4*i]   = fmaf(dA[0], u.x, dKa[4*i]);   dKa[4*i+1] = fmaf(dA[1], u.y, dKa[4*i+1]);
          dKa[4*i+2] = fmaf(dA[0], u.z, dKa[4*i+2]); dKa[4*i+3] = fmaf(dA[1], u.w, dKa[4*i+3]);
          dVa[4*i]   = fmaf(at[0], v.x, dVa[4*i]);   dVa[4*i+1] = fmaf(at[1], v.y, dVa[4*i+1]);
          dVa[4*i+2] = fmaf(at[0], v.z, dVa[4*i+2]); dVa[4*i+3] = fmaf(at[1], v.w, dVa[4*i+3]);
        }
#pragma unroll
        for (int k = 0; k < 8; ++k) { dq[2 * k] = dA[0] * Kf[2 * k]; dq[2 * k + 1] = dA[1] * Kf[2 * k + 1]; }
        a.dqp[(((size_t)b * ntile + mt) * N + l) * 64 + lane] = reduce16_keep_own(dq, p);
      }
      SCHED_FENCE();
      if (!(a.guard & 1))
      {
        float bT[4], bR[4];
#pragma unroll
        for (int s = 0; s < 4; ++s) {
          bT[s] = sc1[(q + 4 * s) * 16 + p];
          bR[s] = (p < 9) ? sc2[(q + 4 * s) * 12 + p] : 0.f;
        }
        {
          const int lb = 64 * q + 4 * ((p >> 2) ^ q) + (p & 3);
          const float* eb = et + lb;
          const float* db = dt + lb;
#pragma unroll
          for (int t = 0; t < G::TILES; ++t)
#pragma unroll
            for (int s = 0; s < 4; ++s) {
              accT[t] = MFMA(elem_read_st<DE>(eb, et, p, q, s, t), bT[s], accT[t]);
              accR[t] = MFMA(elem_read_st<DE>(db, dt, p, q, s, t), bR[s], accR[t]);
            }
        }
      }
      lds_sync();
      SCHED_FENCE();
      if (!(a.guard & 2)) {
        float4 dxh[G::TILES];
        float m1 = 0.f, m2 = 0.f;
        Bf8 gB1, gB2;
        if constexpr (MM != 0) {
          const uint32_t h0 = pk_bf16(dge[0], dge[1]), h1 = pk_bf16(dge[2], dge[3]);
          gB1.u[0] = h0; gB1.u[1] = h1; gB1.u[2] = h0; gB1.u[3] = h1;
          gB2.u[0] = pk_bf16(dge[0] - __uint_as_float(h0 << 16), dge[1] - __uint_as_float(h0 & 0xFFFF0000u));
          gB2.u[1] = pk_bf16(dge[2] - __uint_as_float(h1 << 16), dge[3] - __uint_as_float(h1 & 0xFFFF0000u));
          gB2.u[2] = 0u; gB2.u[3] = 0u;
        }
#pragma unroll
        for (int t = 0; t < G::TILES; ++t) {
          const float4 xh = frag_read<DE>(et, p, q, t);
          v4f d = {0.f, 0.f, 0.f, 0.f};
          if constexpr (MM != 0) {
            Bf8 wa, wb;
            wa.q = *reinterpret_cast<const uint4*>(wsD + (t * 64 + lane) * 4);
            d = MFMA_BF(wa.v, gB1.v, d);
            if (SPLIT) {
              wb.u[0] = wa.u[0]; wb.u[1] = wa.u[1]; wb.u[2] = 0u; wb.u[3] = 0u;
              d = MFMA_BF(wb.v, gB2.v, d);
            }
          } else {
          const float4 w = *reinterpret_cast<const float4*>(wsD + (t * 64 + lane) * 4);
          d = MFMA(w.x, dge[0], d);
          d = MFMA(w.y, dge[1], d);
          d = MFMA(w.z, dge[2], d);
          d = MFMA(w.w, dge[3], d);
          }
          dxh[t] = make_float4(d[0], d[1], d[2], d[3]);
          m1 += (d[0] + d[1]) + (d[2] + d[3]);
          m2 = fmaf(d[0], xh.x, m2); m2 = fmaf(d[1], xh.y, m2);
          m2 = fmaf(d[2], xh.z, m2); m2 = fmaf(d[3], xh.w, m2);
        }
        m1 = sum_over_q(m1) * (1.0f / DE);
        m2 = sum_over_q(m2) * (1.0f / DE);
        if (a.flags & EGT_BF_NO_EDGE_LN) { m1 = 0.f; m2 = 0.f; }
        float* orow = dex_o + (pair0 + p) * DE + 4 * q;
#pragma unroll
        for (int t = 0; t < G::TILES; ++t) {
          if (16 * t + 4 * q < DE) {
            const float4 dyv = frag_read<DE>(dt, p, q, t);
            const float4 xh = frag_read<DE>(et, p, q, t);
            float4 o;
            o.x = dyv.x + rstd * (dxh[t].x - m1 - xh.x * m2);
            o.y = dyv.y + rstd * (dxh[t].y - m1 - xh.y * m2);
            o.z = dyv.z + rstd * (dxh[t].z - m1 - xh.z * m2);
            o.w = dyv.w + rstd * (dxh[t].w - m1 - xh.w * m2);
            if (kvalid) { if (EGT_NT_BWD_ST) egt_st4_nt(orow + 16 * t, o); else *reinterpret_cast<float4*>(orow + 16 * t) = o; }
          }
        }
        lds_sync();
      }
      SCHED_FENCE();
    }
    float4* ko = reinterpret_cast<float4*>(a.dkvp + (((((size_t)b * a.NLR + lr) * N + m) * 2 + 0) * 4 + q) * 16);
    float4* vo = reinterpret_cast<float4*>(a.dkvp + (((((size_t)b * a.NLR + lr) * N + m) * 2 + 1) * 4 + q) * 16);
    if (balance && r1 < nl && r0 == 0) {
      while (pflag[wave + 1] == 0) __builtin_amdgcn_s_sleep(1);
      __builtin_amdgcn_fence(__ATOMIC_ACQUIRE, "workgroup");
      if (kvalid) {
#pragma unroll
        for (int i = 0; i < 4; ++i) {
          const float4 kk = ko[i], vv = vo[i];
          dKa[4*i] += kk.x; dKa[4*i+1] += kk.y; dKa[4*i+2] += kk.z; dKa[4*i+3] += kk.w;
          dVa[4*i] += vv.x; dVa[4*i+1] += vv.y; dVa[4*i+2] += vv.z; dVa[4*i+3] += vv.w;
        }
      }
    }
    if (kvalid) {
#pragma unroll
      for (int i = 0; i < 4; ++i) {
        ko[i] = make_float4(dKa[4*i], dKa[4*i+1], dKa[4*i+2], dKa[4*i+3]);
        vo[i] = make_float4(dVa[4*i], dVa[4*i+1], dVa[4*i+2], dVa[4*i+3]);
      }
    }
    if (balance && r0 > 0) {
      __builtin_amdgcn_fence(__ATOMIC_RELEASE, "workgroup");
      asm volatile("s_waitcnt vmcnt(0)" ::: "memory");
      if (lane == 0) pflag[wave] = 1;
    }
  }
#pragma unroll
  for (int r = 0; r < 4; ++r) ssum[r] = row_sum16(ssum[r]);
  __syncthreads();
  float* ep = sm + wave * G::EP;
#pragma unroll
  for (int t = 0; t < G::TILES; ++t)
#pragma unroll
    for (int r = 0; r < 4; ++r) {
      ep[(16 * t + 4 * q + r) * 16 + p] = accT[t][r];
      ep[G::DEP * 16 + 16 + (16 * t + 4 * q + r) * 16 + p] = accR[t][r];
    }
  if (p == 0) {
#pragma unroll
    for (int r = 0; r < 4; ++r) ep[G::DEP * 16 + 4 * q + r] = ssum[r];
  }
  __syncthreads();
  float* out = a.epart + (size_t)wg * G::EP;
  for (int i = threadIdx.x; i < G::EP; i += 256)
    out[i] = (sm[i] + sm[G::EP + i]) + (sm[2 * G::EP + i] + sm[3 * G::EP + i]);
}

template <int DE, bool BF, int R>
__global__ void __launch_bounds__(256, 2) k_block_bwd_v4r(BlockArgs a) {
  seed_from_device(a);
  using G = Geo<DE>;
  typedef typename EdgeT<BF>::type ET;
  const ET* e_in = reinterpret_cast<const ET*>(a.e);
  const ET* dey_in = reinterpret_cast<const ET*>(a.de_out);
  ET* dex_o = reinterpret_cast<ET*>(a.de);
  extern __shared__ __attribute__((aligned(16))) float sm[];
  const int lane = threadIdx.x & 63, wave = threadIdx.x >> 6;
  const int p = lane & 15, q = lane >> 4;
  const int N = a.N, TL = a.TL;
  const int wg = a.xcd ? egt_xcd_remap(blockIdx.x, gridDim.x) : (int)blockIdx.x;
  int b, lr;
  egt_group_order(wg, a.B, a.NLR, N, b, lr, TL);
  const int l_begin = lr * TL, l_end = min(N, l_begin + TL), nl = l_end - l_begin;
  const bool gated = (a.flags & EGT_BF_GATE) != 0;
  const bool clip = (a.flags & EGT_BF_CLIP) != 0;
  constexpr int TF = G::TILE_FLOATS;
  constexpr int PWR = R * (2 * TF + 256 + 192);
  constexpr int WSLAB = G::TILES * 256;
  float* et0 = sm + wave * PWR;
  float* dt0 = et0 + R * TF;
  float* sc10 = dt0 + R * TF;
  float* sc20 = sc10 + R * 256;
  constexpr int AREA = 4 * PWR > BWD_PRO_WS ? 4 * PWR : BWD_PRO_WS;
  static_assert(4 * G::EP <= AREA, "edge partial staging must fit the LDS tile area");
  float* qd = sm + AREA;
  float* wsA = qd + TL * QD_LD;
  float* wsB = wsA + WSLAB;
  float* wsD = wsB + WSLAB;
  float* park = wsD + WSLAB;
  volatile int* pflag = reinterpret_cast<volatile int*>(park + 3 * 2048);
  if (threadIdx.x < 4) pflag[threadIdx.x] = 0;
  bwd_stage_rows<256, 3>(a, qd, b, l_begin, nl);
  if (a.pro) {
    __syncthreads();
    bwd_node_prologue<DE>(a, sm, qd, b, l_begin, wg);
  }
  for (int i = threadIdx.x; i < G::TILES * 256; i += 256) {
    const int t = i >> 8, ln = (i >> 2) & 63, u = i & 3, pp = ln & 15, qq = ln >> 4;
    const int c = 16 * t + 4 * qq + u;
    wsA[i] = a.pw[c * 16 + pp];
    const int hd = 2 * (pp >> 2) + (pp & 1);
    wsB[i] = ((pp & 2) == 0 && c < DE) ? a.Wr[hd * DE + c] : 0.f;
    wsD[i] = a.pw[(16 * t + pp) * 16 + 4 * qq + u];
  }
  float c2r[4];
#pragma unroll
  for (int r = 0; r < 4; ++r) c2r[r] = a.pw[G::DEP * 16 + 4 * q + r];
  v4f accT[G::TILES], accR[G::TILES];
#pragma unroll
  for (int t = 0; t < G::TILES; ++t) { accT[t] = (v4f){0.f, 0.f, 0.f, 0.f}; accR[t] = (v4f){0.f, 0.f, 0.f, 0.f}; }
  float ssum[4] = {0.f, 0.f, 0.f, 0.f};
  __syncthreads();

  const int ntile = (N + 15) / 16;
  const int npair = (nl + R - 1) / R;
  const bool balance = ntile >= 4 && (ntile & 3) != 0;
  const int TT = ntile * npair;
  const int t0 = balance ? (wave * TT) >> 2 : 0, t1 = balance ? ((wave + 1) * TT) >> 2 : 0;
  const int mt_first = balance ? t0 / npair : wave, mt_last = balance ? (t1 - 1) / npair : ntile - 1, mt_step = balance ? 1 : 4;
  for (int mt = mt_first; mt <= mt_last; mt += mt_step) {
    const int q0 = (balance && mt == mt_first) ? t0 - mt * npair : 0;
    const int q1 = (balance && mt == mt_last) ? t1 - mt * npair : npair;
    const int m0 = mt * 16, m = m0 + p, kv = min(16, N - m0);
    const bool kvalid = m < N;
    float Kf[16], Vf[16], dKa[16], dVa[16];
    const size_t rowm = (size_t)b * N + (kvalid ? m : N - 1);
    {
      const float4* kp = reinterpret_cast<const float4*>(a.qkvp + rowm * QKVP + 64 + q * 16);
      const float4* vp = reinterpret_cast<const float4*>(a.qkvp + rowm * QKVP + 128 + q * 16);
#pragma unroll
      for (int i = 0; i < 4; ++i) {
        const float4 kv = kp[i], vv = vp[i];
        Kf[4*i] = kv.x; Kf[4*i+1] = kv.y; Kf[4*i+2] = kv.z; Kf[4*i+3] = kv.w;
        Vf[4*i] = vv.x; Vf[4*i+1] = vv.y; Vf[4*i+2] = vv.z; Vf[4*i+3] = vv.w;
      }
#pragma unroll
      for (int i = 0; i < 16; ++i) { dKa[i] = 0.f; dVa[i] = 0.f; }
    }
    const float kadd = (a.km && a.km[rowm] == 0) ? -EGT_NEG : 0.0f;
    const MaskRegs mr{make_float2(1.f, 1.f), 0};
    TileRegs<DE> te[R], td[R];
    auto prefetch = [&](int lq) {
#pragma unroll
      for (int i = 0; i < R; ++i) {
        const size_t pair0 = ((size_t)b * N + l_begin + min(R * lq + i, nl - 1)) * N + m0;
        tile_gload<DE>(te[i], e_in + pair0 * DE, lane, kv);
        tile_gload<DE>(td[i], dey_in + pair0 * DE, lane, kv);
      }
    };
    prefetch(q0);
    for (int lq = q0; lq < q1; ++lq) {
      const int lb = l_begin + R * lq;
      const int nr = min(R, nl - R * lq);
      size_t pair0[R];
#pragma unroll
      for (int i = 0; i < R; ++i) pair0[i] = ((size_t)b * N + min(lb + i, l_end - 1)) * N + m0;
      lds_sync();
#pragma unroll
      for (int i = 0; i < R; ++i) {
        tile_lds_put<DE>(et0 + i * TF, te[i], lane, kv);
        tile_lds_put<DE>(dt0 + i * TF, td[i], lane, kv);
      }
      if (lq + 1 < q1) prefetch(lq + 1);
      lds_sync();
      float rstd[R];
      v4f acc[R], dhx[R];
#pragma unroll
      for (int i = 0; i < R; ++i) {
        if (i >= nr) continue;
        float* et = et0 + i * TF;
        const float* dt = dt0 + i * TF;
        acc[i] = (v4f){c2r[0], c2r[1], c2r[2], c2r[3]};
        dhx[i] = (v4f){0.f, 0.f, 0.f, 0.f};
        float4 x[G::TILES];
#pragma unroll
        for (int t = 0; t < G::TILES; ++t) x[t] = frag_read<DE>(et, p, q, t);
        rstd[i] = ln_frags<DE>(x, q, a.ln_eps, (a.flags & EGT_BF_NO_EDGE_LN) == 0);
#pragma unroll
        for (int t = 0; t < G::TILES; ++t) {
          frag_write<DE>(et, p, q, t, x[t]);
          const float4 w = *reinterpret_cast<const float4*>(wsA + (t * 64 + lane) * 4);
          acc[i] = MFMA(w.x, x[t].x, acc[i]);
          acc[i] = MFMA(w.y, x[t].y, acc[i]);
          acc[i] = MFMA(w.z, x[t].z, acc[i]);
          acc[i] = MFMA(w.w, x[t].w, acc[i]);
          const float4 dyv = frag_read<DE>(dt, p, q, t);
          const float4 wb = *reinterpret_cast<const float4*>(wsB + (t * 64 + lane) * 4);
          dhx[i] = MFMA(wb.x, dyv.x, dhx[i]);
          dhx[i] = MFMA(wb.y, dyv.y, dhx[i]);
          dhx[i] = MFMA(wb.z, dyv.z, dhx[i]);
          dhx[i] = MFMA(wb.w, dyv.w, dhx[i]);
        }
      }
      float dge[R][4], dA[R][2], at[R][2];
#pragma unroll
      for (int i = 0; i < R; ++i) {
        if (i >= nr) continue;
        const float* qr = qd + (R * lq + i) * QD_LD;
        float dots[2], dAd[2], hh[2];
        {
          const float4* qp = reinterpret_cast<const float4*>(qr + q * 16);
          const float4* dp = reinterpret_cast<const float4*>(qr + 64 + q * 16);
          float d0 = 0.f, d1 = 0.f, e0 = 0.f, e1 = 0.f;
#pragma unroll
          for (int u4 = 0; u4 < 4; ++u4) {
            const float4 u = qp[u4], v = dp[u4];
            d0 = fmaf(u.x, Kf[4*u4], d0);   d1 = fmaf(u.y, Kf[4*u4+1], d1);
            d0 = fmaf(u.z, Kf[4*u4+2], d0); d1 = fmaf(u.w, Kf[4*u4+3], d1);
            e0 = fmaf(v.x, Vf[4*u4], e0);   e1 = fmaf(v.y, Vf[4*u4+1], e1);
            e0 = fmaf(v.z, Vf[4*u4+2], e0); e1 = fmaf(v.w, Vf[4*u4+3], e1);
          }
          dots[0] = d0; dots[1] = d1; dAd[0] = e0; dAd[1] = e1;
        }
        const float4* sp = reinterpret_cast<const float4*>(qr + 128 + q * 8);
        const float4 s0 = sp[0], s1 = sp[1];
        const float st[8] = {s0.x, s0.y, s0.z, 0.f, s1.x, s1.y, s1.z, 0.f};
        float xl[2], gl[2], inr[2];
#pragma unroll
        for (int j = 0; j < 2; ++j) {
          const float araw = dots[j] * a.scale;
          float ah = araw;
          inr[j] = 1.0f;
          if (clip) {
            inr[j] = (araw >= a.clip_lo && araw <= a.clip_hi) ? 1.0f : 0.0f;
            ah = fminf(fmaxf(araw, a.clip_lo), a.clip_hi);
          }
          hh[j] = ah + acc[i][2 * j + 1];
          xl[j] = hh[j];
          gl[j] = acc[i][2 * j];
        }
        apply_masks<false>(a, kadd, mr, (pair0[i] + p) * BH, q, xl, gl);
        if (!kvalid) { xl[0] = xl[1] = -3.0e38f; gl[0] = gl[1] = -3.0e38f; }
#pragma unroll
        for (int j = 0; j < 2; ++j) {
          const float S = __expf(xl[j] - st[4 * j]) * st[4 * j + 1];
          const float g = gated ? egt_sigmoid(gl[j]) : 1.0f;
          const float dS = dAd[j] * g;
          const float dGl = gated ? dAd[j] * S * g * (1.0f - g) : 0.f;
          const float dH = S * (dS - st[4 * j + 2]) + dhx[i][j];
          dA[i][j] = dH * inr[j] * a.scale;
          at[i][j] = S * g;
          dge[i][2 * j] = dGl;
          dge[i][2 * j + 1] = dH;
        }
#pragma unroll
        for (int r = 0; r < 4; ++r) ssum[r] += dge[i][r];
        float* sc1 = sc10 + i * 256;
        float* sc2 = sc20 + i * 192;
        *reinterpret_cast<float4*>(sc1 + p * 16 + 4 * q) = make_float4(dge[i][0], dge[i][1], dge[i][2], dge[i][3]);
        *reinterpret_cast<float2*>(sc2 + p * 12 + 2 * q) = make_float2(hh[0], hh[1]);
        if (q == 0) sc2[p * 12 + 8] = 1.0f;
        SCHED_FENCE();
      }
      lds_sync();
#pragma unroll
      for (int i = 0; i < R; ++i) {
        if (i >= nr) continue;
        const float* qr = qd + (R * lq + i) * QD_LD;
        const float4* qp = reinterpret_cast<const float4*>(qr + q * 16);
        const float4* dp = reinterpret_cast<const float4*>(qr + 64 + q * 16);
        float dq[16];
#pragma unroll
        for (int u4 = 0; u4 < 4; ++u4) {
          const float4 u = qp[u4], v = dp[u4];
          dKa[4*u4]   = fmaf(dA[i][0], u.x, dKa[4*u4]);   dKa[4*u4+1] = fmaf(dA[i][1], u.y, dKa[4*u4+1]);
          dKa[4*u4+2] = fmaf(dA[i][0], u.z, dKa[4*u4+2]); dKa[4*u4+3] = fmaf(dA[i][1], u.w, dKa[4*u4+3]);
          dVa[4*u4]   = fmaf(at[i][0], v.x, dVa[4*u4]);   dVa[4*u4+1] = fmaf(at[i][1], v.y, dVa[4*u4+1]);
          dVa[4*u4+2] = fmaf(at[i][0], v.z, dVa[4*u4+2]); dVa[4*u4+3] = fmaf(at[i][1], v.w, dVa[4*u4+3]);
        }
#pragma unroll
        for (int k = 0; k < 8; ++k) { dq[2 * k] = dA[i][0] * Kf[2 * k]; dq[2 * k + 1] = dA[i][1] * Kf[2 * k + 1]; }
        a.dqp[(((size_t)b * ntile + mt) * N + lb + i) * 64 + lane] = reduce16_keep_own(dq, p);
        const float* et = et0 + i * TF;
        const float* dt = dt0 + i * TF;
        const float* sc1 = sc10 + i * 256;
        const float* sc2 = sc20 + i * 192;
        float bT[4], bR[4];
#pragma unroll
        for (int s4 = 0; s4 < 4; ++s4) {
          bT[s4] = sc1[(q + 4 * s4) * 16 + p];
          bR[s4] = (p < 9) ? sc2[(q + 4 * s4) * 12 + p] : 0.f;
        }
#pragma unroll
        for (int t = 0; t < G::TILES; ++t)
#pragma unroll
          for (int s4 = 0; s4 < 4; ++s4) {
            accT[t] = MFMA(elem_read<DE>(et, q + 4 * s4, 16 * t + p), bT[s4], accT[t]);
            accR[t] = MFMA(elem_read<DE>(dt, q + 4 * s4, 16 * t + p), bR[s4], accR[t]);
          }
        SCHED_FENCE();
      }
      lds_sync();
      float4 dxh[R][G::TILES];
      float m1[R], m2[R];
#pragma unroll
      for (int i = 0; i < R; ++i) {
        if (i >= nr) continue;
        const float* et = et0 + i * TF;
        float s1 = 0.f, s2 = 0.f;
#pragma unroll
        for (int t = 0; t < G::TILES; ++t) {
          const float4 w = *reinterpret_cast<const float4*>(wsD + (t * 64 + lane) * 4);
          const float4 xh = frag_read<DE>(et, p, q, t);
          v4f d = {0.f, 0.f, 0.f, 0.f};
          d = MFMA(w.x, dge[i][0], d);
          d = MFMA(w.y, dge[i][1], d);
          d = MFMA(w.z, dge[i][2], d);
          d = MFMA(w.w, dge[i][3], d);
          dxh[i][t] = make_float4(d[0], d[1], d[2], d[3]);
          s1 += (d[0] + d[1]) + (d[2] + d[3]);
          s2 = fmaf(d[0], xh.x, s2); s2 = fmaf(d[1], xh.y, s2);
          s2 = fmaf(d[2], xh.z, s2); s2 = fmaf(d[3], xh.w, s2);
        }
        m1[i] = sum_over_q(s1) * (1.0f / DE);
        m2[i] = sum_over_q(s2) * (1.0f / DE);
        if (a.flags & EGT_BF_NO_EDGE_LN) { m1[i] = 0.f; m2[i] = 0.f; }
      }
      lds_sync();
#pragma unroll
      for (int i = 0; i < R; ++i) {
        if (i >= nr) continue;
        const float* et = et0 + i * TF;
        float* dt = dt0 + i * TF;
#pragma unroll
        for (int t = 0; t < G::TILES; ++t) {
          const float4 dyv = frag_read<DE>(dt, p, q, t);
          const float4 xh = frag_read<DE>(et, p, q, t);
          float4 o;
          o.x = dyv.x + rstd[i] * (dxh[i][t].x - m1[i] - xh.x * m2[i]);
          o.y = dyv.y + rstd[i] * (dxh[i][t].y - m1[i] - xh.y * m2[i]);
          o.z = dyv.z + rstd[i] * (dxh[i][t].z - m1[i] - xh.z * m2[i]);
          o.w = dyv.w + rstd[i] * (dxh[i][t].w - m1[i] - xh.w * m2[i]);
          frag_write<DE>(dt, p, q, t, o);
        }
      }
      lds_sync();
#pragma unroll
      for (int i = 0; i < R; ++i)
        if (i < nr) tile_from_lds<DE>(dt0 + i * TF, dex_o + pair0[i] * DE, lane, kv);
    }
    if (q0 > 0) {
      float* pk = park + (wave - 1) * 2048 + lane;
#pragma unroll
      for (int i = 0; i < 16; ++i) { pk[i * 64] = dKa[i]; pk[(16 + i) * 64] = dVa[i]; }
      asm volatile("s_waitcnt lgkmcnt(0)" ::: "memory");
      if (lane == 0) pflag[wave] = 1;
    } else {
      if (q1 < npair) {
        while (pflag[wave + 1] == 0) __builtin_amdgcn_s_sleep(1);
        asm volatile("" ::: "memory");
        const float* pk = park + wave * 2048 + lane;
#pragma unroll
        for (int i = 0; i < 16; ++i) { dKa[i] += pk[i * 64]; dVa[i] += pk[(16 + i) * 64]; }
      }
      float4* ko = reinterpret_cast<float4*>(a.dkvp + (((((size_t)b * a.NLR + lr) * N + m) * 2 + 0) * 4 + q) * 16);
      float4* vo = reinterpret_cast<float4*>(a.dkvp + (((((size_t)b * a.NLR + lr) * N + m) * 2 + 1) * 4 + q) * 16);
      if (kvalid) {
#pragma unroll
        for (int i = 0; i < 4; ++i) {
          ko[i] = make_float4(dKa[4*i], dKa[4*i+1], dKa[4*i+2], dKa[4*i+3]);
          vo[i] = make_float4(dVa[4*i], dVa[4*i+1], dVa[4*i+2], dVa[4*i+3]);
        }
      }
    }
  }
#pragma unroll
  for (int r = 0; r < 4; ++r) ssum[r] = row_sum16(ssum[r]);
  __syncthreads();
  float* ep = sm + wave * G::EP;
#pragma unroll
  for (int t = 0; t < G::TILES; ++t)
#pragma unroll
    for (int r = 0; r < 4; ++r) {
      ep[(16 * t + 4 * q + r) * 16 + p] = accT[t][r];
      ep[G::DEP * 16 + 16 + (16 * t + 4 * q + r) * 16 + p] = accR[t][r];
    }
  if (p == 0) {
#pragma unroll
    for (int r = 0; r < 4; ++r) ep[G::DEP * 16 + 4 * q + r] = ssum[r];
  }
  __syncthreads();
  float* out = a.epart + (size_t)wg * G::EP;
  for (int i = threadIdx.x; i < G::EP; i += 256)
    out[i] = (sm[i] + sm[G::EP + i]) + (sm[2 * G::EP + i] + sm[3 * G::EP + i]);
}
```

### egt_amd/csrc/egt_block_dev.h

```cpp
#pragma once
#include "egt_block.h"
#include "egt_tile.h"

template <int DE>
__device__ __forceinline__ v4f project(const float4 (&x)[Geo<DE>::TILES],
                                       const float (&wA)[4 * Geo<DE>::TILES], v4f acc) {
  using G = Geo<DE>;
#pragma unroll
  for (int t = 0; t < G::TILES; ++t) {
    acc = MFMA(wA[4 * t + 0], x[t].x, acc);
    acc = MFMA(wA[4 * t + 1], x[t].y, acc);
    acc = MFMA(wA[4 * t + 2], x[t].z, acc);
    acc = MFMA(wA[4 * t + 3], x[t].w, acc);
  }
  return acc;

}

struct MaskRegs { float2 mv; unsigned short rb; };

__device__ __forceinline__ void seed_from_device(BlockArgs& a) {
  if (a.sd) { a.s0 ^= a.sd[0]; a.s1 ^= a.sd[1]; }
}

template <bool ML>
__device__ __forceinline__ void mask_gload(const BlockArgs& a, MaskRegs& mr, size_t pairc, int q) {
  if (!ML) return;
  if (a.M) mr.mv = *reinterpret_cast<const float2*>(a.M + pairc * BH + 2 * q);
  if (a.rm) mr.rb = *reinterpret_cast<const unsigned short*>(a.rm + pairc * BH + 2 * q);
}

template <bool ML>
__device__ __forceinline__ void apply_masks(const BlockArgs& a, float kadd, const MaskRegs& mr,
                                            size_t idx8, int q, float (&x)[2], float (&gl)[2]) {
#pragma unroll
  for (int j = 0; j < 2; ++j) {
    float xv = x[j], gv = gl[j];
    if (a.km) { xv += kadd; gv += kadd; }
    if (ML && a.M) {
      const float mm = ((j ? mr.mv.y : mr.mv.x) - 1.0f) * EGT_NEG;
      xv += mm; gv += mm;
    }
    if ((ML && a.rm) || a.rng_rm) {
      bool hit;
      if (ML && a.rm) hit = ((mr.rb >> (8 * j)) & 0xFF) != 0;
      else hit = (egt_hash32((uint32_t)(idx8 + 2 * q + j), a.s0, a.s1) >> 8) < a.rm_thr;
      const float mrv = hit ? -EGT_NEG : 0.0f;
      xv += mrv; gv += mrv;
    }
    x[j] = xv; gl[j] = gv;
  }
}

__device__ __forceinline__ float reduce16_keep_own(const float (&v)[16], int p) {
  float t0, t1, t2, t3, t4, t5, t6, t7, u0, u1, u2, u3;
  asm volatile(
      "s_nop 1\n\t"
      "v_add_f32_dpp %0, %8, %8 row_ror:8 row_mask:0xf bank_mask:0xf\n\t"
      "v_add_f32_dpp %1, %9, %9 row_ror:8 row_mask:0xf bank_mask:0xf\n\t"
      "v_add_f32_dpp %2, %10, %10 row_ror:8 row_mask:0xf bank_mask:0xf\n\t"
      "v_add_f32_dpp %3, %11, %11 row_ror:8 row_mask:0xf bank_mask:0xf\n\t"
      "v_add_f32_dpp %4, %12, %12 row_ror:8 row_mask:0xf bank_mask:0xf\n\t"
      "v_add_f32_dpp %5, %13, %13 row_ror:8 row_mask:0xf bank_mask:0xf\n\t"
      "v_add_f32_dpp %6, %14, %14 row_ror:8 row_mask:0xf bank_mask:0xf\n\t"
      "v_add_f32_dpp %7, %15, %15 row_ror:8 row_mask:0xf bank_mask:0xf\n\t"
      "v_add_f32_dpp %0, %16, %16 row_ror:8 row_mask:0xf bank_mask:0xc\n\t"
      "v_add_f32_dpp %1, %17, %17 row_ror:8 row_mask:0xf bank_mask:0xc\n\t"
      "v_add_f32_dpp %2, %18, %18 row_ror:8 row_mask:0xf bank_mask:0xc\n\t"
      "v_add_f32_dpp %3, %19, %19 row_ror:8 row_mask:0xf bank_mask:0xc\n\t"
      "v_add_f32_dpp %4, %20, %20 row_ror:8 row_mask:0xf bank_mask:0xc\n\t"
      "v_add_f32_dpp %5, %21, %21 row_ror:8 row_mask:0xf bank_mask:0xc\n\t"
      "v_add_f32_dpp %6, %22, %22 row_ror:8 row_mask:0xf bank_mask:0xc\n\t"
      "v_add_f32_dpp %7, %23, %23 row_ror:8 row_mask:0xf bank_mask:0xc"
      : "=&v"(t0), "=&v"(t1), "=&v"(t2), "=&v"(t3), "=&v"(t4), "=&v"(t5), "=&v"(t6), "=&v"(t7)
      : "v"(v[0]), "v"(v[1]), "v"(v[2]), "v"(v[3]), "v"(v[4]), "v"(v[5]), "v"(v[6]), "v"(v[7]),
        "v"(v[8]), "v"(v[9]), "v"(v[10]), "v"(v[11]), "v"(v[12]), "v"(v[13]), "v"(v[14]), "v"(v[15]));
  asm volatile(
      "s_nop 1\n\t"
      "v_add_f32_dpp %0, %4, %4 row_ror:12 row_mask:0xf bank_mask:0x5\n\t"
      "v_add_f32_dpp %1, %5, %5 row_ror:12 row_mask:0xf bank_mask:0x5\n\t"
      "v_add_f32_dpp %2, %6, %6 row_ror:12 row_mask:0xf bank_mask:0x5\n\t"
      "v_add_f32_dpp %3, %7, %7 row_ror:12 row_mask:0xf bank_mask:0x5\n\t"
      "v_add_f32_dpp %0, %8, %8 row_ror:4 row_mask:0xf bank_mask:0xa\n\t"
      "v_add_f32_dpp %1, %9, %9 row_ror:4 row_mask:0xf bank_mask:0xa\n\t"
      "v_add_f32_dpp %2, %10, %10 row_ror:4 row_mask:0xf bank_mask:0xa\n\t"
      "v_add_f32_dpp %3, %11, %11 row_ror:4 row_mask:0xf bank_mask:0xa"
      : "=&v"(u0), "=&v"(u1), "=&v"(u2), "=&v"(u3)
      : "v"(t0), "v"(t1), "v"(t2), "v"(t3), "v"(t4), "v"(t5), "v"(t6), "v"(t7));
  const float w4[4] = {u0, u1, u2, u3};
  float w2[2];
  const bool b1 = (p & 2) != 0, b0 = (p & 1) != 0;
#pragma unroll
  for (int i = 0; i < 2; ++i) {
    const float snd = b1 ? w4[i] : w4[i + 2], kp = b1 ? w4[i + 2] : w4[i];
    w2[i] = kp + lane_xor<2>(snd);
  }
  const float snd = b0 ? w2[0] : w2[1], kp = b0 ? w2[1] : w2[0];
  return kp + lane_xor<1>(snd);
}

#define KV_LD 132
#define QS_LD 68

template <int NT>
__device__ __forceinline__ void fwd_stage_kv(float* kvs, const float* kvsrc, int N) {
  for (int base = 0; base < N * 32; base += 8 * NT) {
    float4 kvb[8];
#pragma unroll
    for (int u = 0; u < 8; ++u) {
      const int i = base + threadIdx.x + NT * u, row = min(i >> 5, N - 1), f = i & 31;
      kvb[u] = *reinterpret_cast<const float4*>(kvsrc + (size_t)row * QKVP + 64 + f * 4);
    }
#pragma unroll
    for (int u = 0; u < 8; ++u) {
      const int i = base + threadIdx.x + NT * u, row = i >> 5, f = i & 31;
      if (i < N * 32) *reinterpret_cast<float4*>(kvs + row * KV_LD + f * 4) = kvb[u];
    }
  }
}

struct FwdEpiRegs { float wo[16], wq[3][16], bo, hres[4]; };
template <bool D64>
__device__ __forceinline__ void fwd_epilogue_load(const BlockArgs& a, FwdEpiRegs& R, int b, int l0, int N, int wave, int p, int q) {
    const int Dh = D64 ? 64 : a.Dh;
    float (&wo)[16] = R.wo; float (&wq)[3][16] = R.wq;
    const int c = wave * 16 + p;
    const bool cok = D64 || c < Dh;
    {
      const int ln = 16 * q + p;
      const float4* fwo = reinterpret_cast<const float4*>(a.wfrag + WFRAG_FWO) + wave * 256 + ln;
#pragma unroll
      for (int s4 = 0; s4 < 4; ++s4) {
        const float4 v = fwo[s4 * 64];
        wo[4 * s4] = v.x; wo[4 * s4 + 1] = v.y; wo[4 * s4 + 2] = v.z; wo[4 * s4 + 3] = v.w;
      }
      if (a.epi == 2) {
        const float4* fwq = reinterpret_cast<const float4*>(a.nx_wfrag + WFRAG_FWQ) + wave * 768 + ln;
#pragma unroll
        for (int j = 0; j < 3; ++j)
#pragma unroll
          for (int s4 = 0; s4 < 4; ++s4) {
            const float4 v = fwq[(j * 4 + s4) * 64];
            wq[j][4 * s4] = v.x; wq[j][4 * s4 + 1] = v.y; wq[j][4 * s4 + 2] = v.z; wq[j][4 * s4 + 3] = v.w;
          }
      }
    }
    R.bo = cok ? a.bo[c] : 0.f;
#pragma unroll
    for (int r = 0; r < 4; ++r) R.hres[r] = cok ? a.h[((size_t)b * N + min(l0 + 4 * q + r, N - 1)) * Dh + c] : 0.f;
}
template <bool D64>
__device__ __forceinline__ void fwd_epilogue_compute(const BlockArgs& a, const FwdEpiRegs& R, float* sm, float* qs, int b, int l0, int nrows, int N,
                                                     int wave, int p, int q) {
    const int Dh = D64 ? 64 : a.Dh;
    const float (&wo)[16] = R.wo; const float (&wq)[3][16] = R.wq; const float (&hres)[4] = R.hres;
    const float bo = R.bo;
    const int c = wave * 16 + p;
    const bool cok = D64 || c < Dh;
    __syncthreads();
    float* hs = sm;
    v4f acc = {bo, bo, bo, bo};
#pragma unroll
    for (int s = 0; s < 16; ++s) acc = MFMA(qs[p * QS_LD + 4 * s + q], wo[s], acc);
#pragma unroll
    for (int r = 0; r < 4; ++r) {
      const int row = 4 * q + r, l = l0 + row;
      const float hv = acc[r] + hres[r];
      if (row < nrows && cok) a.h_out[((size_t)b * N + l) * Dh + c] = hv;
      hs[row * QS_LD + c] = hv;
    }
    if (a.epi == 2) {
      __syncthreads();
      {
        float* x = hs + (4 * wave + q) * QS_LD;
        const float inv = D64 ? 1.0f / 64 : 1.0f / (float)Dh;
        float v[4], sm1 = 0.f;
#pragma unroll
        for (int i = 0; i < 4; ++i) { v[i] = x[p + 16 * i]; sm1 += v[i]; }
        const float mu = row_sum16(sm1) * inv;
        float ss = 0.f;
#pragma unroll
        for (int i = 0; i < 4; ++i) { v[i] = (D64 || p + 16 * i < Dh) ? v[i] - mu : 0.f; ss = fmaf(v[i], v[i], ss); }
        const float rstd = rsqrtf(row_sum16(ss) * inv + a.ln_eps);
#pragma unroll
        for (int i = 0; i < 4; ++i) {
          const int ci = p + 16 * i;
          const bool ok = D64 || ci < Dh;
          x[ci] = ok ? fmaf(v[i] * rstd, a.nx_nm_g[ci], a.nx_nm_b[ci]) : 0.f;
        }
      }
      __syncthreads();
#pragma unroll
      for (int j = 0; j < 3; ++j) {
        const int cq = (wave + 4 * j) * 16 + p;
        const float bq = (D64 || (cq & 63) < Dh) ? a.nx_bqkv[(cq >> 6) * Dh + (cq & 63)] : 0.f;
        v4f aq = {bq, bq, bq, bq};
#pragma unroll
        for (int s = 0; s < 16; ++s) aq = MFMA(hs[p * QS_LD + 4 * s + q], wq[j][s], aq);
        const int sx = cq >> 6, cc = cq & 63, kk = cc >> 3, hh = cc & 7;
        const int pos = sx * 64 + (hh >> 1) * 16 + kk * 2 + (hh & 1);
#pragma unroll
        for (int r = 0; r < 4; ++r) {
          const int l = l0 + 4 * q + r;
          if (4 * q + r < nrows) a.nx_qkvp[((size_t)b * N + l) * QKVP + pos] = aq[r];
        }
      }
    }
  }
template <bool D64>
__device__ __forceinline__ void fwd_node_epilogue_t(const BlockArgs& a, float* sm, float* qs, int b, int l0, int nrows, int N,
                                                    int wave, int p, int q) {
  FwdEpiRegs R;
  fwd_epilogue_load<D64>(a, R, b, l0, N, wave, p, q);
  fwd_epilogue_compute<D64>(a, R, sm, qs, b, l0, nrows, N, wave, p, q);
}
__device__ __forceinline__ void fwd_node_epilogue(const BlockArgs& a, float* sm, float* qs, int b, int l0, int nrows, int N,
                                                  int wave, int p, int q) {
  if (a.Dh == 64) fwd_node_epilogue_t<true>(a, sm, qs, b, l0, nrows, N, wave, p, q);
  else fwd_node_epilogue_t<false>(a, sm, qs, b, l0, nrows, N, wave, p, q);
}
__device__ __forceinline__ void fwd_node_epilogue_load(const BlockArgs& a, FwdEpiRegs& R, int b, int l0, int N, int wave, int p, int q) {
  if (a.Dh == 64) fwd_epilogue_load<true>(a, R, b, l0, N, wave, p, q);
  else fwd_epilogue_load<false>(a, R, b, l0, N, wave, p, q);
}
__device__ __forceinline__ void fwd_node_epilogue_finish(const BlockArgs& a, const FwdEpiRegs& R, float* sm, float* qs, int b, int l0, int nrows, int N,
                                                         int wave, int p, int q) {
  if (a.Dh == 64) fwd_epilogue_compute<true>(a, R, sm, qs, b, l0, nrows, N, wave, p, q);
  else fwd_epilogue_compute<false>(a, R, sm, qs, b, l0, nrows, N, wave, p, q);
}

__device__ __forceinline__ void fwd_node_epilogue_idle(const BlockArgs& a) {
  __syncthreads();
  if (a.epi == 2) { __syncthreads(); __syncthreads(); }
}

#define QD_LD 160
#define SCHED_FENCE() __builtin_amdgcn_sched_barrier(0)

template <int NT, int NU>
__device__ __forceinline__ void bwd_stage_rows(const BlockArgs& a, float* qd, int b, int l_begin, int nl) {
  float4 sv[NU];
#pragma unroll
  for (int u = 0; u < NU; ++u) {
    const int i = threadIdx.x + NT * u, r = i / 40, f = i % 40;
    const bool ok = i < nl * 40 && !(a.pro && f >= 16 && f < 32);
    const size_t rowl = (size_t)b * a.N + l_begin + (ok ? r : 0);
    const float* src = f < 16 ? a.qkvp + rowl * QKVP + f * 4
                     : f < 32 ? a.dvp + rowl * 64 + (f - 16) * 4
                              : a.stats + rowl * 32 + (f - 32) * 4;
    sv[u] = ok ? *reinterpret_cast<const float4*>(src) : make_float4(0.f, 0.f, 0.f, 0.f);
  }
#pragma unroll
  for (int u = 0; u < NU; ++u) {
    const int i = threadIdx.x + NT * u, r = i / 40, f = i % 40;
    if (i < nl * 40 && !(a.pro && f >= 16 && f < 32)) {
      float4 v = sv[u];
      if (f >= 32) v.y = 1.0f / v.y;
      *reinterpret_cast<float4*>(qd + r * QD_LD + f * 4) = v;
    }
  }
}

#define EGT_PRO_UNROLL 4
#define BWD_PRO_WS 8192
struct BwdProRegs { float4 hx, gq[3], wq[12], wo[4]; float dho[4], gmm[4], va[4]; };

#define BWD_PRO_COMMON()                                                                                   \
  constexpr int LD = 68, LD3 = 196;                                                                        \
  const int t = threadIdx.x, lane = t & 63, wave = __builtin_amdgcn_readfirstlane(t >> 6);                        \
  const int p = lane & 15, q = lane >> 4, N = a.N;                                                         \
  const size_t row0 = (size_t)b * N + l_begin;                                                             \
  const int lnrow = 4 * wave + q;                \
                                     \
  const int nv = min(a.TL, N - l_begin);                      \
  auto rc = [&](int r) { return row0 + max(min(r, nv - 1), 0); };                  \
  const int Dh = D64 ? 64 : a.Dh;                                                                          \
  (void)LD; (void)LD3; (void)lnrow; (void)p; (void)q; (void)rc; (void)Dh

template <int DE, bool D64>
__device__ __forceinline__ void bwd_prologue_load_wo_va(const BlockArgs& a, int b, int l_begin, BwdProRegs& R) {
  BWD_PRO_COMMON();
  const bool iok = D64 || 16 * wave + p < Dh;
#pragma unroll
  for (int s = 0; s < 4; ++s)
    R.wo[s] = reinterpret_cast<const float4*>(a.wfrag + WFRAG_BWO)[(wave * 4 + s) * 64 + lane];
#pragma unroll
  for (int r = 0; r < 4; ++r) R.va[r] = iok ? a.v_att[rc(4 * q + r) * Dh + 16 * wave + p] : 0.f;
}
template <int DE, bool D64>
__device__ __forceinline__ void bwd_prologue_load_main(const BlockArgs& a, int b, int l_begin, BwdProRegs& R) {
  BWD_PRO_COMMON();
    const float4 z4 = make_float4(0.f, 0.f, 0.f, 0.f);
    R.hx = (D64 || (t & 15) * 4 < Dh) ? *reinterpret_cast<const float4*>(a.up_h + rc(t >> 4) * Dh + (t & 15) * 4) : z4;
#pragma unroll
    for (int i = 0; i < 4; ++i) {
      const bool ok = D64 || p + 16 * i < Dh;
      R.dho[i] = ok ? a.up_dh_out[rc(lnrow) * Dh + p + 16 * i] : 0.f;
      R.gmm[i] = ok ? a.up_nm_g[p + 16 * i] : 0.f;
    }
    {
      const float* base[3]; size_t pstride[3]; int NPu[3];
#pragma unroll
      for (int u = 0; u < 3; ++u) {
        const int i = t + u * 256, r = i / 48, pos4 = (i % 48) * 4, sx = pos4 >> 6;
        const int rr = max(min(r, nv - 1), 0);
        NPu[u] = sx == 0 ? a.NQP : a.NLR;
        base[u] = sx == 0 ? a.up_dqp + ((size_t)b * NPu[u] * N + l_begin + rr) * 64 + pos4
                          : a.up_dkvp + (((size_t)b * NPu[u] * N + l_begin + rr) * 2 + (sx - 1)) * 64 + (pos4 & 63);
        pstride[u] = sx == 0 ? (size_t)N * 64 : (size_t)N * 128;
        R.gq[u] = z4;
      }
      const int NPm = max(a.NQP, a.NLR);
      for (int p0 = 0; p0 < NPm; p0 += EGT_PRO_UNROLL) {
        float4 w[3][EGT_PRO_UNROLL];
#pragma unroll
        for (int u = 0; u < 3; ++u)
#pragma unroll
          for (int j = 0; j < EGT_PRO_UNROLL; ++j)
            w[u][j] = *reinterpret_cast<const float4*>(base[u] + (size_t)max(min(p0 + j, NPu[u] - 1), 0) * pstride[u]);
#pragma unroll
        for (int u = 0; u < 3; ++u)
#pragma unroll
          for (int j = 0; j < EGT_PRO_UNROLL; ++j) {
            const bool in = p0 + j < NPu[u];
            R.gq[u].x += in ? w[u][j].x : 0.f; R.gq[u].y += in ? w[u][j].y : 0.f;
            R.gq[u].z += in ? w[u][j].z : 0.f; R.gq[u].w += in ? w[u][j].w : 0.f;
          }
      }
#pragma unroll
      for (int u = 0; u < 3; ++u)
        if ((t + u * 256) / 48 >= nv) R.gq[u] = z4;
    }
#pragma unroll
    for (int s = 0; s < 12; ++s)
      R.wq[s] = reinterpret_cast<const float4*>(a.up_wfrag + WFRAG_BWQ)[(wave * 12 + s) * 64 + lane];
}

template <int DE, bool D64>
__device__ __forceinline__ void bwd_prologue_compute(const BlockArgs& a, float* ws, float* qd, int b, int l_begin, int wg, BwdProRegs& R) {
  float* dqs = ws;
  float* xs = dqs + 16 * 196;
  float* dls = xs + 16 * 68;
  float* dhs = dls + 16 * 68;
  float* rs = dhs + 16 * 68;
  float* dlp = rs + 16;
  static_assert(16 * 196 + 3 * 16 * 68 + 16 + 4 * 16 * 8 <= BWD_PRO_WS, "prologue scratch");
  BWD_PRO_COMMON();
  float4 (&wo)[4] = R.wo;
  float (&va)[4] = R.va;
  if (a.pro == 2) {
    float4 (&gq)[3] = R.gq; float4 (&wq)[12] = R.wq; float (&dho)[4] = R.dho; float (&gmm)[4] = R.gmm; const float4 hx = R.hx;
    *reinterpret_cast<float4*>(xs + (t >> 4) * LD + (t & 15) * 4) = hx;
#pragma unroll
    for (int u = 0; u < 3; ++u) {
      const int i = t + u * 256, r = i / 48, pos4 = (i % 48) * 4, sx = pos4 >> 6;
      const int qq = (pos4 >> 4) & 3, k0 = (pos4 >> 1) & 7;
      float* d = dqs + r * LD3 + sx * 64 + k0 * 8 + 2 * qq;
      const bool k0ok = D64 || k0 * 8 < Dh, k1ok = D64 || (k0 + 1) * 8 < Dh;
      d[0] = k0ok ? gq[u].x : 0.f; d[1] = k0ok ? gq[u].y : 0.f; d[8] = k1ok ? gq[u].z : 0.f; d[9] = k1ok ? gq[u].w : 0.f;
    }
    __syncthreads();
    const float invD = D64 ? 1.0f / 64 : 1.0f / (float)Dh;
    {
      float* xr = xs + lnrow * LD;
      float v[4], s1 = 0.f;
#pragma unroll
      for (int i = 0; i < 4; ++i) { v[i] = xr[p + 16 * i]; s1 += v[i]; }
      const float mu = row_sum16(s1) * invD;
      float ss = 0.f;
#pragma unroll
      for (int i = 0; i < 4; ++i) { v[i] = (D64 || p + 16 * i < Dh) ? v[i] - mu : 0.f; ss = fmaf(v[i], v[i], ss); }
      const float rstd = rsqrtf(row_sum16(ss) * invD + a.ln_eps);
#pragma unroll
      for (int i = 0; i < 4; ++i) xr[p + 16 * i] = v[i] * rstd;
      if (p == 0) rs[lnrow] = rstd;
    }
    {
      v4f acc = {0.f, 0.f, 0.f, 0.f};
      const float* ar = dqs + p * LD3 + 48 * q;
#pragma unroll
      for (int s = 0; s < 12; ++s) {
        const float4 av = *reinterpret_cast<const float4*>(ar + 4 * s);
        acc = MFMA(av.x, wq[s].x, acc);
        acc = MFMA(av.y, wq[s].y, acc);
        acc = MFMA(av.z, wq[s].z, acc);
        acc = MFMA(av.w, wq[s].w, acc);
      }
#pragma unroll
      for (int r = 0; r < 4; ++r) dls[(4 * q + r) * LD + 16 * wave + p] = acc[r];
    }
    for (int i = t; i < nv * 48; i += 256) {
      const int r = i / 48, c4 = (i % 48) * 4;
      if (D64 || (c4 & 63) < Dh)
        *reinterpret_cast<float4*>(a.up_dqkv_sv + (row0 + r) * (3 * Dh) + (c4 >> 6) * Dh + (c4 & 63)) = *reinterpret_cast<const float4*>(dqs + r * LD3 + c4);
    }
    __syncthreads();
    {
      const float* xr = xs + lnrow * LD;
      const float* dl = dls + lnrow * LD;
      float dx[4], m1 = 0.f, m2 = 0.f;
#pragma unroll
      for (int i = 0; i < 4; ++i) {
        dx[i] = dl[p + 16 * i] * gmm[i];
        m1 += dx[i];
        m2 = fmaf(dx[i], xr[p + 16 * i], m2);
      }
      m1 = row_sum16(m1) * invD;
      m2 = row_sum16(m2) * invD;
      const float rstd = rs[lnrow];
      float* dh_out_rw = const_cast<float*>(a.dh_out);
#pragma unroll
      for (int i = 0; i < 4; ++i) {
        const int c = p + 16 * i;
        const bool ok = lnrow < nv && (D64 || c < Dh);
        const float dv = ok ? dho[i] + rstd * (dx[i] - m1 - xr[c] * m2) : 0.f;
        if (ok) dh_out_rw[(row0 + lnrow) * Dh + c] = dv;
        dhs[lnrow * LD + c] = dv;
      }
    }
    {
      float* sp = a.up_spart + (size_t)wg * (5 * Dh);
      if (t < 192) {
        float s0 = 0.f, s1 = 0.f;
#pragma unroll
        for (int r = 0; r < 16; r += 2) { s0 += dqs[r * LD3 + t]; s1 += dqs[(r + 1) * LD3 + t]; }
        if ((D64 || (t & 63) < Dh) && nv > 0) sp[(t >> 6) * Dh + (t & 63)] = s0 + s1;
      } else {
        const int c = t - 192;
        float g0 = 0.f, b0 = 0.f;
#pragma unroll
        for (int r = 0; r < 16; ++r) { const float d0 = dls[r * LD + c]; g0 = fmaf(d0, xs[r * LD + c], g0); b0 += d0; }
        if ((D64 || c < Dh) && nv > 0) {
          sp[3 * Dh + c] = g0;
          sp[4 * Dh + c] = b0;
        }
      }
    }
  } else {
    const bool ok = (t >> 4) < nv && (D64 || (t & 15) * 4 < Dh);
    const float4 dv4 = ok ? *reinterpret_cast<const float4*>(a.dh_out + rc(t >> 4) * Dh + (t & 15) * 4) : make_float4(0.f, 0.f, 0.f, 0.f);
    *reinterpret_cast<float4*>(dhs + (t >> 4) * LD + (t & 15) * 4) =
        make_float4(ok ? dv4.x : 0.f, ok ? dv4.y : 0.f, ok ? dv4.z : 0.f, ok ? dv4.w : 0.f);
  }
  bwd_prologue_load_wo_va<DE, D64>(a, b, l_begin, R);
  __syncthreads();
  {
    v4f acc = {0.f, 0.f, 0.f, 0.f};
    const float* ar = dhs + p * LD + 16 * q;
#pragma unroll
    for (int s = 0; s < 4; ++s) {
      const float4 av = *reinterpret_cast<const float4*>(ar + 4 * s);
      acc = MFMA(av.x, wo[s].x, acc);
      acc = MFMA(av.y, wo[s].y, acc);
      acc = MFMA(av.z, wo[s].z, acc);
      acc = MFMA(av.w, wo[s].w, acc);
    }
    const int i = 16 * wave + p, k = i >> 3, hh = i & 7;
    const int pos = (hh >> 1) * 16 + k * 2 + (hh & 1);
#pragma unroll
    for (int r = 0; r < 4; ++r) {
      const int row = 4 * q + r;
      if (row < nv) qd[row * QD_LD + 64 + pos] = acc[r];
      float pr = acc[r] * va[r];
      pr += lane_xor<8>(pr);
      if (p < 8) dlp[(wave * 16 + row) * 8 + p] = pr;
    }
  }
  if (t < 64) {
    float s0 = 0.f, s1 = 0.f;
#pragma unroll
    for (int r = 0; r < 16; r += 2) { s0 += dhs[r * LD + t]; s1 += dhs[(r + 1) * LD + t]; }
    if ((D64 || t < Dh) && nv > 0) a.sbo[(size_t)wg * Dh + t] = s0 + s1;
  }
  __syncthreads();
  if (t < 128 && (t >> 3) < nv) {
    const int row = t >> 3, hd = t & 7;
    qd[row * QD_LD + 128 + hd * 4 + 2] = (dlp[(0 * 16 + row) * 8 + hd] + dlp[(1 * 16 + row) * 8 + hd]) +
                                         (dlp[(2 * 16 + row) * 8 + hd] + dlp[(3 * 16 + row) * 8 + hd]);
  }
}

template <int DE, bool D64>
__device__ __forceinline__ void bwd_node_prologue_t(const BlockArgs& a, float* ws, float* qd, int b, int l_begin, int wg) {
  BwdProRegs R;
  if (a.pro == 2) bwd_prologue_load_main<DE, D64>(a, b, l_begin, R);
  bwd_prologue_compute<DE, D64>(a, ws, qd, b, l_begin, wg, R);
}
template <int DE>
__device__ __forceinline__ void bwd_node_prologue_load(const BlockArgs& a, BwdProRegs& R, int b, int l_begin) {
  if (a.pro != 2) return;
  if (a.Dh == 64) bwd_prologue_load_main<DE, true>(a, b, l_begin, R);
  else bwd_prologue_load_main<DE, false>(a, b, l_begin, R);
}
template <int DE>
__device__ __forceinline__ void bwd_node_prologue_finish(const BlockArgs& a, float* ws, float* qd, int b, int l_begin, int wg, BwdProRegs& R) {
  if (a.Dh == 64) bwd_prologue_compute<DE, true>(a, ws, qd, b, l_begin, wg, R);
  else bwd_prologue_compute<DE, false>(a, ws, qd, b, l_begin, wg, R);
}
__device__ __forceinline__ void bwd_node_prologue_idle(const BlockArgs& a) {
  if (a.pro == 2) { __syncthreads(); __syncthreads(); }
  __syncthreads();
  __syncthreads();
}
template <int DE>
__device__ __forceinline__ void bwd_node_prologue(const BlockArgs& a, float* ws, float* qd, int b, int l_begin, int wg) {
  if (a.Dh == 64) bwd_node_prologue_t<DE, true>(a, ws, qd, b, l_begin, wg);
  else bwd_node_prologue_t<DE, false>(a, ws, qd, b, l_begin, wg);
}
```

### include/egt_amd.h

```cpp
#ifndef EGT_AMD_H_
#define EGT_AMD_H_

#include <stddef.h>
#include <stdint.h>

#ifdef __cplusplus
extern "C" {
#endif

#define EGT_ABI_VERSION 4

#define EGT_OK 0
#define EGT_E_NULL (-1)
#define EGT_E_SHAPE (-2)
#define EGT_E_DTYPE (-3)
#define EGT_E_FLAGS (-4)
#define EGT_E_HIP (-5)
#define EGT_E_WORKSPACE (-6)
#define EGT_E_RCCL (-7)

#define EGT_F32 0
#define EGT_BF16 1

#define EGT_F_EDGE_INPUT 0x001u
#define EGT_F_GATE_INPUT 0x002u
#define EGT_F_ATTN_MASK 0x004u
#define EGT_F_SCALE_DEGREE 0x008u
#define EGT_F_SCALER_LINEAR 0x010u
#define EGT_F_TRAINING 0x020u
#define EGT_F_CLIP 0x040u

typedef struct egt_attn_desc {
  int32_t B, N, H, d;
  int32_t dtype;
  uint32_t flags;
  float clip_lo, clip_hi;
  float random_mask_prob;
  float attn_dropout;
  int32_t num_virtual_nodes;
  int32_t reserved;
  uint64_t seed;
} egt_attn_desc;
#define EGT_ATTN_WS_SHARED 0x1

const char* egt_last_error_string(void);
int egt_abi_version(void);

int egt_attn_fwd(const egt_attn_desc* desc, const void* qkv, const void* E,
                 const void* G, const uint8_t* key_mask, const void* attn_mask,
                 const uint8_t* rand_mask, const uint8_t* drop_keep, void* v_att,
                 void* h_hat, void* a_tild, void* rowstats, void* stream);

size_t egt_attn_bwd_workspace_bytes(const egt_attn_desc* desc);
int egt_attn_bwd(const egt_attn_desc* desc, const void* qkv, const void* E,
                 const void* G, const uint8_t* key_mask, const void* attn_mask,
                 const uint8_t* rand_mask, const uint8_t* drop_keep,
                 const void* v_att, const void* rowstats, const void* d_v_att,
                 const void* d_h_ext, void* d_qkv, void* d_E, void* d_G,
                 void* workspace, void* stream);

int egt_attn_mfma_supported(const egt_attn_desc* desc, int need_a_tild);
size_t egt_attn_mfma_fwd_workspace_bytes(const egt_attn_desc* desc);
size_t egt_attn_mfma_workspace_bytes(const egt_attn_desc* desc);
int egt_attn_mfma_fwd(const egt_attn_desc* desc, const void* qkv, const void* E,
                      const void* G, const uint8_t* key_mask, const void* attn_mask,
                      const uint8_t* rand_mask, void* v_att, void* h_hat, void* rowstats,
                      void* workspace, void* stream);
int egt_attn_mfma_bwd(const egt_attn_desc* desc, const void* qkv, const void* E,
                      const void* G, const uint8_t* key_mask, const void* attn_mask,
                      const uint8_t* rand_mask, const void* v_att, void* rowstats,
                      const void* d_v_att, const void* d_h_ext, void* d_qkv, void* d_E,
                      void* d_G, void* workspace, void* stream);

int egt_mask_sample(int which, uint64_t seed, float prob, int32_t B, int32_t N,
                    int32_t H, uint8_t* out, void* stream);

int egt_seed_advance(uint64_t* words, int32_t count, uint64_t increment, void* stream);

#define EGT_EP_LAYERNORM 0x1u
#define EGT_EP_GATES 0x2u
#define EGT_ACT_NONE 0
#define EGT_ACT_LRELU 1
#define EGT_ACT_RELU 2
#define EGT_ACT_ELU 3

typedef struct egt_edge_desc {
  int64_t rows;
  int32_t De, H;
  int32_t dtype;
  uint32_t flags;
  int32_t act;
  float act_alpha;
  float ln_eps;
  int32_t reserved;
} egt_edge_desc;

int egt_edge_proj_fwd(const egt_edge_desc* desc, const void* e,
                      const void* ln_gamma, const void* ln_beta, const void* Wg,
                      const void* bg, const void* We, const void* be,
                      void* G_out, void* E_out, void* stream);

size_t egt_edge_proj_bwd_workspace_bytes(const egt_edge_desc* desc);
int egt_edge_proj_bwd(const egt_edge_desc* desc, const void* e,
                      const void* ln_gamma, const void* ln_beta, const void* Wg,
                      const void* We, const void* E_out, const void* d_G,
                      const void* d_E, void* d_e, void* d_ln_gamma,
                      void* d_ln_beta, void* d_Wg, void* d_bg, void* d_We,
                      void* d_be, void* workspace, void* stream);
int egt_edge_proj_bwd_acc(const egt_edge_desc* desc, const void* e,
                          const void* ln_gamma, const void* ln_beta, const void* Wg,
                          const void* We, const void* E_out, const void* d_G,
                          const void* d_E, const void* d_e_base, void* d_e,
                          void* d_ln_gamma, void* d_ln_beta, void* d_Wg, void* d_bg,
                          void* d_We, void* d_be, void* workspace, void* stream);

int egt_edge_update_fwd(const egt_edge_desc* desc, const void* e,
                        const void* h_hat, const void* Wr, const void* br,
                        void* e_out, void* stream);

size_t egt_edge_update_bwd_workspace_bytes(const egt_edge_desc* desc);
int egt_edge_update_bwd(const egt_edge_desc* desc, const void* d_e_out,
                        const void* h_hat, const void* Wr, void* d_h_hat,
                        void* d_Wr, void* d_br, void* workspace, void* stream);

#define EGT_BF_GATE 0x1u
#define EGT_BF_ATTN_MASK 0x2u
#define EGT_BF_TRAINING 0x4u
#define EGT_BF_CLIP 0x8u
#define EGT_BF_NO_EDGE_LN 0x10u
#define EGT_BF_SEED_DEVICE 0x20u
#define EGT_BF_STATIC_EDGE 0x40u

typedef struct egt_block_desc {
  int32_t B, N, H, d, De;
  int32_t dtype;
  uint32_t flags;
  float clip_lo, clip_hi;
  float random_mask_prob;
  float ln_eps;
  int32_t reserved;
  uint64_t seed;
  const void* seed_device;
} egt_block_desc;

typedef struct egt_block_params {
  const void* norm_edge_gamma;
  const void* norm_edge_beta;
  const void* attention_gates_kernel;
  const void* attention_gates_bias;
  const void* dense_edge_b_kernel;
  const void* dense_edge_b_bias;
  const void* norm_mha_gamma;
  const void* norm_mha_beta;
  const void* dense_qkv_kernel;
  const void* dense_qkv_bias;
  const void* dense_mha_kernel;
  const void* dense_mha_bias;
  const void* dense_edge_r_kernel;
  const void* dense_edge_r_bias;
} egt_block_params;

int egt_block_supported(const egt_block_desc* desc);
const char* egt_block_bwd_kernel(const egt_block_desc* desc);
const char* egt_block_launch_form(const egt_block_desc* desc);
size_t egt_block_saved_bytes(const egt_block_desc* desc);
size_t egt_block_workspace_bytes(const egt_block_desc* desc);

int egt_block_fwd(const egt_block_desc* desc, const egt_block_params* params,
                  const void* h, const void* e, const uint8_t* key_mask,
                  const void* attn_mask, const uint8_t* rand_mask, void* h_out,
                  void* e_out, void* saved, void* workspace, void* stream);

int egt_block_bwd(const egt_block_desc* desc, const egt_block_params* params,
                  const void* h, const void* e, const uint8_t* key_mask,
                  const void* attn_mask, const uint8_t* rand_mask,
                  const void* saved, const void* d_h_out, const void* d_e_out,
                  void* d_h, void* d_e, const egt_block_params* grads,
                  void* workspace, void* stream);

size_t egt_stack_saved_bytes(const egt_block_desc* desc, int32_t layers);
size_t egt_stack_workspace_bytes(const egt_block_desc* desc, int32_t layers);
int egt_stack_fwd(const egt_block_desc* desc, int32_t layers,
                  const egt_block_params* params, const void* h, const void* e,
                  const uint8_t* key_mask, const void* attn_mask, void* h_out,
                  void* e_out, void* saved, void* workspace, void* stream);
int egt_stack_bwd(const egt_block_desc* desc, int32_t layers,
                  const egt_block_params* params, const void* h, const void* e,
                  const uint8_t* key_mask, const void* attn_mask, const void* saved,
                  const void* d_h_out, const void* d_e_out, void* d_h, void* d_e,
                  const egt_block_params* grads, void* workspace, void* stream);

int egt_pair_supported(const egt_block_desc* desc);
size_t egt_pair_workspace_bytes(const egt_block_desc* desc);
int egt_pair_fwd(const egt_block_desc* desc, const egt_block_params* params, const void* qkv,
                 const void* e, const uint8_t* key_mask, void* v_att, void* e_out, void* rowstats,
                 void* workspace, void* stream);
int egt_pair_bwd(const egt_block_desc* desc, const egt_block_params* params, const void* qkv,
                 const void* e, const uint8_t* key_mask, const void* v_att, void* rowstats,
                 const void* d_v_att, const void* d_e_out, void* d_qkv, void* d_e,
                 const egt_block_params* grads, void* workspace, void* stream);

#define EGT_MM_F32 0
#define EGT_MM_BF16X3 1
#define EGT_MM_BF16 2

typedef struct egt_ffn_desc {
  int64_t rows;
  int32_t width;
  int32_t dtype;
  int32_t activation;
  float ln_eps;
  int32_t matmul;
  int32_t flags;
} egt_ffn_desc;
#define EGT_FFN_WS_PREPARED 1

typedef struct egt_ffn_params {
  const void* norm_gamma;
  const void* norm_beta;
  const void* lr1_kernel;
  const void* lr1_bias;
  const void* lr2_kernel;
  const void* lr2_bias;
} egt_ffn_params;

int egt_ffn_supported(const egt_ffn_desc* desc);
size_t egt_ffn_workspace_bytes(const egt_ffn_desc* desc);
int egt_ffn_fwd(const egt_ffn_desc* desc, const egt_ffn_params* params, const void* x, void* y,
                void* workspace, void* stream);
int egt_ffn_bwd(const egt_ffn_desc* desc, const egt_ffn_params* params, const void* x,
                const void* dy, void* dx, const egt_ffn_params* grads, void* workspace,
                void* stream);

int egt_node_mask_from_features(const int32_t* features, int32_t B, int32_t N, int32_t num_virtual_nodes,
                                uint8_t* mask, void* stream);
int egt_node_mask_from_float_features(const float* features, int32_t B, int32_t N, int32_t width,
                                      float mask_value, int32_t num_virtual_nodes, uint8_t* mask,
                                      void* stream);
int egt_constrained_edge_mask(const float* adj, int32_t B, int32_t N, int32_t H, int32_t num_virtual_nodes,
                              float* M, void* stream);

typedef struct egt_embed_desc {
  int32_t B, N, De;
  int32_t upto_hop;
  int32_t clip_hops;
  int32_t num_edge_features;
  int32_t dtype;
  int32_t num_float_features;
  float mask_value;
  int32_t reserved;
} egt_embed_desc;
int egt_edge_embed_supported(const egt_embed_desc* desc);
size_t egt_edge_embed_hops_bytes(const egt_embed_desc* desc);
size_t egt_edge_embed_workspace_bytes(const egt_embed_desc* desc);
int egt_edge_embed_fwd(const egt_embed_desc* desc, const int32_t* feature_matrix, const void* graph_matrix,
                       const void* float_features , const void* fm_table,
                       const void* adj_kernel, const void* adj_bias, void* hops, void* e_out, void* stream);
int egt_edge_embed_bwd(const egt_embed_desc* desc, const int32_t* feature_matrix, const void* hops,
                       const void* d_e, void* d_fm_table, void* d_adj_kernel, void* d_adj_bias,
                       void* workspace, void* stream);

#define EGT_EH_LAYERNORM 0x1
typedef struct egt_head_desc {
  int32_t B, N, De, M0, M1, C;
  int32_t dtype;
  int32_t activation;
  int32_t flags;
  float ln_eps;
  int32_t reserved;
} egt_head_desc;

typedef struct egt_head_params {
  void* edge_norm_final_gamma;
  void* edge_norm_final_beta;
  void* mlp_out_dist_targ_0_kernel;
  void* mlp_out_dist_targ_0_bias;
  void* mlp_out_dist_targ_1_kernel;
  void* mlp_out_dist_targ_1_bias;
  void* distance_target_kernel;
  void* distance_target_bias;
} egt_head_params;

int egt_distance_target(const float* adj, int32_t B, int32_t N, int32_t T, uint8_t* target, void* stream);
int egt_edge_head_supported(const egt_head_desc* desc);
size_t egt_edge_head_workspace_bytes(const egt_head_desc* desc);
int egt_edge_head_fwd(const egt_head_desc* desc, const egt_head_params* params, const void* e, const uint8_t* target,
                      float* per_graph_loss , void* workspace, void* stream);
int egt_edge_head_bwd(const egt_head_desc* desc, const egt_head_params* params, const void* e, const uint8_t* target,
                      const float* d_per_graph , void* d_e, const egt_head_params* grads, void* workspace,
                      void* stream);

#define EGT_DP_ID_BYTES 128
int egt_dp_unique_id(void* id_out );
int egt_dp_init(const void* id , int32_t world, int32_t rank);
int egt_dp_allreduce(void* buf, size_t count, int32_t average, void* stream);
int egt_dp_world(void);
int egt_dp_rank(void);
int egt_dp_finalize(void);

int egt_prof_enable(int on);
int egt_prof_filter(const char* kernel_name);
int egt_prof_stride(int every);
int egt_prof_read(const char* name, int64_t* count, double* total_ms);
int egt_prof_collect_graph(int reset_counts);
int egt_prof_forget_graphs(void);
int egt_prof_names(char* buf, size_t cap);

#ifdef __cplusplus
}
#endif
#endif
```

Baseline: 79470 graphs/s.

## Run v5 backward with 512-thread workgroups covering two 16-row halves

Adds a two-half mode to the v5 backward kernel. Each 512-thread workgroup handles 32 query rows as two 16-row halves, so the key/value tiles and weight slabs are staged once and shared, and the dK/dV partials of half 1 are parked in LDS and summed by half 0 before being written. It is enabled by default when N is a multiple of 32, TL is 16 and there are enough workgroups, which halves the workgroup count and the partial-reduction work. In exchange it needs more LDS per workgroup, limits occupancy to one block per launch bound, and adds extra barriers inside each tile iteration.

```diff
diff --git a/egt_amd/_lib.py b/egt_amd/_lib.py
--- a/egt_amd/_lib.py
+++ b/egt_amd/_lib.py
@@ -156,6 +156,7 @@
     "egt_block_supported": (C.c_int, [C.POINTER(BlockDesc)]),
     "egt_block_bwd_kernel": (C.c_char_p, [C.POINTER(BlockDesc)]),
     "egt_block_launch_form": (C.c_char_p, [C.POINTER(BlockDesc)]),
+    "egt_block_bwd_rows": (C.c_int, [C.POINTER(BlockDesc)]),
     "egt_block_saved_bytes": (C.c_size_t, [C.POINTER(BlockDesc)]),
     "egt_block_workspace_bytes": (C.c_size_t, [C.POINTER(BlockDesc)]),
     "egt_block_fwd": (C.c_int, [C.POINTER(BlockDesc), C.POINTER(BlockParams)] + [_VP] * 10),
diff --git a/egt_amd/csrc/egt_block.hip b/egt_amd/csrc/egt_block.hip
--- a/egt_amd/csrc/egt_block.hip
+++ b/egt_amd/csrc/egt_block.hip
@@ -21,6 +21,7 @@
   int bwd_mm;
   int bwd_tl, fwd_rows;
   int nrw_fwd_waves, nrw_bwd_waves, nrw_fwd_half;
+  int bwd_wg32;
 };
 static bool env_flag_raw(const char* name) {
   const char* v = getenv(name);
@@ -42,6 +43,7 @@
     v.nrw_fwd_waves = env_int("EGT_NRW_FWD_WAVES", 0);
     v.nrw_bwd_waves = env_int("EGT_NRW_BWD_WAVES", 0);
     v.nrw_fwd_half = env_int("EGT_NRW_FWD_HALF", -1);
+    v.bwd_wg32 = env_int("EGT_BWD_WG32", -1);
     return v;
   }();
   return e;
@@ -101,6 +103,7 @@
   EgtLaunch bl;
   int bwd_nw;
   int mm;
+  bool wg32;
   int TL, NLR, nwg_bwd, EP;
   size_t v_att, stats, qkvp, pw_sv, wfrag_sv, saved_total;
   size_t dvp, dqp, dkvp, dqp_sz, dkvp_sz, common_total;
@@ -173,6 +176,13 @@
     P.bwd = BwdKernel::v5;
     P.mm = E.bwd_mm;
     P.bl = {P.nwg_bwd, 256, ((size_t)V5_AREA(DE) + (size_t)BWD_TL * QD_LD + 3 * ((GG::TILES + 1) / 2) * 512 + 4) * 4};
+    if constexpr (DE >= 32) {
+      const bool tl_forced = E.bwd_tl >= 4 && E.bwd_tl <= BWD_TL;
+      P.wg32 = (N % 32) == 0 && E.bwd_wg32 != 0 &&
+               (E.bwd_wg32 == 1 || (P.TL == 16 && !tl_forced && (long long)B * (N / 16) >= 2ll * cus));
+      if (P.wg32)
+        P.bl = {B * (N / 32), 512, ((size_t)V5_AREA2(DE) + (size_t)2 * BWD_TL * QD_LD + 3 * ((GG::TILES + 1) / 2) * 512 + 4) * 4};
+    }
   } else {
     constexpr int PW = 3 * GG::TILE_FLOATS + 256 + 192;
     P.bwd = BwdKernel::v4;
@@ -239,12 +249,19 @@
   a.spart_n = a.sbo_n = a.B * ((a.N + NODE_RC - 1) / NODE_RC);
   a.ered = wl + P.ered; a.dqkv_sv = wl + P.dqkv;
   a.TL = P.TL; a.NLR = P.NLR; a.NQP = 1;
+  if (P.wg32) { a.TL = 16; a.NLR = a.N / 32; }
   a.xcd = 1;
 }
 
 extern "C" const char* egt_block_bwd_kernel(const egt_block_desc* d) {
   if (block_check(d, false)) return nullptr;
   return g_bwd_kernel_name[(int)plan_block(d, mask_tensor(d, nullptr)).bwd];
+}
+
+extern "C" int egt_block_bwd_rows(const egt_block_desc* d) {
+  if (block_check(d, false)) return 0;
+  const BlockPlan P = plan_block(d, mask_tensor(d, nullptr));
+  return P.wg32 ? 32 : P.TL;
 }
 
 extern "C" const char* egt_block_launch_form(const egt_block_desc* d) {
@@ -336,7 +353,10 @@
 }
 template <int DE>
 static void launch_v5(BlockArgs& a, const BlockPlan& P, hipStream_t st) {
-  if (P.mm == EGT_MM_BF16X3) {
+  if (P.wg32) {
+    if (P.mm == EGT_MM_BF16X3) egt_launch_planned<k_block_bwd_v5<DE, EGT_MM_BF16X3 | EGT_V5_H2, false>>("k_block_bwd", P.bl, st, a);
+    else egt_launch_planned<k_block_bwd_v5<DE, EGT_MM_F32 | EGT_V5_H2, false>>("k_block_bwd", P.bl, st, a);
+  } else if (P.mm == EGT_MM_BF16X3) {
     if (P.full) egt_launch_planned<k_block_bwd_v5<DE, EGT_MM_BF16X3, false>>("k_block_bwd", P.bl, st, a);
     else egt_launch_planned<k_block_bwd_v5<DE, EGT_MM_BF16X3, true>>("k_block_bwd", P.bl, st, a);
   } else {
@@ -377,13 +397,14 @@
   static_assert(DE % 16 == 0 || DE == 8, "edge widths of the pair kernels");
   const bool pro = fuse;
   a.pro = 0;
+  const int npro = P.wg32 ? a.B * (a.N / 16) : P.nwg_bwd;
   if (pro) {
     a.pro = top ? 1 : 2;
-    a.sbo_n = P.nwg_bwd;
+    a.sbo_n = npro;
     if (!top) {
       a.up_h = above->h; a.up_nm_g = above->nm_g; a.up_Wqkv = above->Wqkv; a.up_wfrag = above->wfrag; a.up_dh_out = above->dh_out;
       a.up_dqp = above->dqp; a.up_dkvp = above->dkvp; a.up_dqkv_sv = above->dqkv_sv; a.up_spart = above->spart;
-      above->spart_n = P.nwg_bwd;
+      above->spart_n = npro;
     }
     if (a.prep) egt_node_launch_prep(&a, 1, st);
   } else if (top) {
@@ -546,7 +567,7 @@
   a.dh = (float*)d_h; a.de = (float*)d_e;
   DISPATCH_BDE(desc->De, launch_bwd<DE>(a, P, (hipStream_t)stream, true, nullptr, nullptr, node_fused_ok(a)));
   egt_node_launch_wgrads(&a, 1, (hipStream_t)stream);
-  egt_node_launch_reduce(&a, 1, P.nwg_bwd, P.EP, (hipStream_t)stream);
+  egt_node_launch_reduce(&a, 1, P.bl.grid, P.EP, (hipStream_t)stream);
   EGT_HIP_LAUNCH_CHECK("egt_block_bwd");
   return EGT_OK;
 }
@@ -613,7 +634,7 @@
                                           l + 1 < layers ? &as[l + 1] : nullptr, fuse));
   }
   egt_node_launch_wgrads(as, layers, (hipStream_t)stream);
-  egt_node_launch_reduce(as, layers, P.nwg_bwd, P.EP, (hipStream_t)stream);
+  egt_node_launch_reduce(as, layers, P.bl.grid, P.EP, (hipStream_t)stream);
   EGT_HIP_LAUNCH_CHECK("egt_stack_bwd");
   return EGT_OK;
 }
diff --git a/egt_amd/csrc/egt_block_bwd.h b/egt_amd/csrc/egt_block_bwd.h
--- a/egt_amd/csrc/egt_block_bwd.h
+++ b/egt_amd/csrc/egt_block_bwd.h
@@ -296,8 +296,14 @@
 
 #define V5_AREA(DE_) ((4 * (3 * Geo<DE_>::TILE_FLOATS + 448) > 4 * Geo<DE_>::TILE_FLOATS + BWD_PRO_WS) \
                           ? 4 * (3 * Geo<DE_>::TILE_FLOATS + 448) : 4 * Geo<DE_>::TILE_FLOATS + BWD_PRO_WS)
-template <int DE, int MM, bool RAG>
-__global__ void __launch_bounds__(256, 2) k_block_bwd_v5(BlockArgs a) {
+#define V5_AREA2(DE_) ((8 * (3 * Geo<DE_>::TILE_FLOATS + 448) > 8 * Geo<DE_>::TILE_FLOATS + 2 * BWD_PRO_WS) \
+                           ? 8 * (3 * Geo<DE_>::TILE_FLOATS + 448) : 8 * Geo<DE_>::TILE_FLOATS + 2 * BWD_PRO_WS)
+#define EGT_V5_H2 4
+template <int DE, int MODE, bool RAG>
+__global__ void __launch_bounds__((MODE & EGT_V5_H2) ? 512 : 256, (MODE & EGT_V5_H2) ? 1 : 2) k_block_bwd_v5(BlockArgs a) {
+  constexpr int MM = MODE & ~EGT_V5_H2, H = (MODE & EGT_V5_H2) ? 2 : 1;
+  static_assert(H == 1 || !RAG, "two halves: N is a multiple of 32");
+  constexpr int NT = 256 * H;
   seed_from_device(a);
   constexpr bool SPLIT = MM == EGT_MM_BF16X3;
   constexpr int NS = (Geo<DE>::TILES + 1) / 2;
@@ -307,28 +313,32 @@
   const float* dey_in = a.de_out;
   float* dex_o = a.de;
   extern __shared__ __attribute__((aligned(16))) float sm[];
-  const int lane = threadIdx.x & 63, wave = __builtin_amdgcn_readfirstlane(threadIdx.x >> 6);
+  const int lane = threadIdx.x & 63, wvw = __builtin_amdgcn_readfirstlane(threadIdx.x >> 6);
+  const int wave = H == 2 ? wvw & 3 : wvw, half = H == 2 ? wvw >> 2 : 0;
+  const int tid = H == 2 ? (int)(threadIdx.x & 255) : (int)threadIdx.x;
   const int p = lane & 15, q = lane >> 4;
   const int N = a.N, TL = a.TL;
   const int wg = a.xcd ? egt_xcd_remap(blockIdx.x, gridDim.x) : (int)blockIdx.x;
   const int b = wg / a.NLR, lr = wg % a.NLR;
-  const int l_begin = lr * TL, l_end = min(N, l_begin + TL), nl = l_end - l_begin;
+  const int l_begin = H == 2 ? lr * 32 + half * 16 : lr * TL, l_end = min(N, l_begin + TL), nl = l_end - l_begin;
+  const int wgp = H == 2 ? 2 * wg + half : wg;
   const bool gated = (a.flags & EGT_BF_GATE) != 0;
   const bool clip = (a.flags & EGT_BF_CLIP) != 0;
   constexpr int PW = 3 * G::TILE_FLOATS + 256 + 192;
   constexpr int WSLAB = (MM != 0 && NS * 512 > G::TILES * 256) ? NS * 512 : G::TILES * 256;
   constexpr int PW2 = 2 * G::TILE_FLOATS + 256 + 192;
-  float* et0 = sm + wave * G::TILE_FLOATS;
-  float* et1 = sm + 4 * G::TILE_FLOATS + wave * PW2;
+  float* et0 = sm + wvw * G::TILE_FLOATS;
+  float* et1 = sm + 4 * H * G::TILE_FLOATS + wvw * PW2;
   const int estr = __builtin_amdgcn_readfirstlane((int)(et1 - et0));
   float* dt = et1 + G::TILE_FLOATS;
   float* sc1 = dt + G::TILE_FLOATS;
   float* sc2 = sc1 + 256;
-  constexpr int AREA = V5_AREA(DE);
-  static_assert(4 * PW == 4 * G::TILE_FLOATS + 4 * PW2 && AREA >= 4 * PW && AREA >= 4 * G::TILE_FLOATS + BWD_PRO_WS, "tile area");
-  float* pro_ws = sm + 4 * G::TILE_FLOATS;
-  float* qd = sm + AREA;
-  float* wsA = qd + TL * QD_LD;
+  constexpr int AREA = H == 2 ? V5_AREA2(DE) : V5_AREA(DE);
+  static_assert(4 * PW == 4 * G::TILE_FLOATS + 4 * PW2 && AREA >= 4 * H * PW && AREA >= 4 * H * G::TILE_FLOATS + H * BWD_PRO_WS, "tile area");
+  static_assert(H == 1 || (AREA >= 8 * G::EP && AREA >= 4 * 2048), "H = 2: the eight edge partials / the parked dK, dV of half 1 fit the tile area");
+  float* pro_ws = sm + 4 * H * G::TILE_FLOATS + half * BWD_PRO_WS;
+  float* qd = sm + AREA + half * (BWD_TL * QD_LD);
+  float* wsA = sm + AREA + (H == 2 ? 2 * BWD_TL : TL) * QD_LD;
   float* wsB = wsA + WSLAB;
   float* wsD = wsB + WSLAB;
   volatile int* pflag = reinterpret_cast<volatile int*>(wsD + WSLAB);
@@ -365,7 +375,7 @@
     float4 sv[3];
 #pragma unroll
     for (int u = 0; u < 3; ++u) {
-      const int i = threadIdx.x + 256 * u, r = i / 40, f = i % 40;
+      const int i = tid + 256 * u, r = i / 40, f = i % 40;
       const bool ok = i < nl * 40 && !(a.pro && f >= 16 && f < 32);
       const size_t rowl = (size_t)b * N + l_begin + (ok ? r : 0);
       const float* src = f < 16 ? a.qkvp + rowl * QKVP + f * 4
@@ -373,22 +383,24 @@
                                 : a.stats + rowl * 32 + (f - 32) * 4;
       sv[u] = ok ? *reinterpret_cast<const float4*>(src) : make_float4(0.f, 0.f, 0.f, 0.f);
     }
-    float sA[G::TILES], sB[G::TILES], sD[G::TILES];
+    constexpr int NSL = (G::TILES + H - 1) / H;
+    float sA[NSL], sB[NSL], sD[NSL];
     if constexpr (MM == 0) {
 #pragma unroll
-      for (int t = 0; t < G::TILES; ++t) {
-        const int i = threadIdx.x + 256 * t, ln = (i >> 2) & 63, u = i & 3, pp = ln & 15, qq = ln >> 4;
+      for (int k = 0; k < NSL; ++k) {
+        const int i = threadIdx.x + NT * k, t = H == 2 ? min(i >> 8, G::TILES - 1) : k;
+        const int ln = (i >> 2) & 63, u = i & 3, pp = ln & 15, qq = ln >> 4;
         const int c = 16 * t + 4 * qq + u;
         const int hd = 2 * (pp >> 2) + (pp & 1);
-        sA[t] = a.pw[c * 16 + pp];
-        sB[t] = ((pp & 2) == 0 && c < DE) ? a.Wr[hd * DE + c] : 0.f;
-        sD[t] = a.pw[(16 * t + pp) * 16 + 4 * qq + u];
-      }
-    }
-    if (a.pro) bwd_node_prologue_load<DE>(a, proR, b, l_begin);
+        sA[k] = a.pw[c * 16 + pp];
+        sB[k] = ((pp & 2) == 0 && c < DE) ? a.Wr[hd * DE + c] : 0.f;
+        sD[k] = a.pw[(16 * t + pp) * 16 + 4 * qq + u];
+      }
+    }
+    if (a.pro) bwd_node_prologue_load<DE, H == 2>(a, proR, b, l_begin);
 #pragma unroll
     for (int u = 0; u < 3; ++u) {
-      const int i = threadIdx.x + 256 * u, r = i / 40, f = i % 40;
+      const int i = tid + 256 * u, r = i / 40, f = i % 40;
       if (i < nl * 40 && !(a.pro && f >= 16 && f < 32)) {
         float4 v = sv[u];
         if (f >= 32) v.y = 1.0f / v.y;
@@ -397,15 +409,15 @@
     }
     if constexpr (MM == 0) {
 #pragma unroll
-      for (int t = 0; t < G::TILES; ++t) {
-        const int i = threadIdx.x + 256 * t;
-        wsA[i] = sA[t]; wsB[i] = sB[t]; wsD[i] = sD[t];
+      for (int k = 0; k < NSL; ++k) {
+        const int i = threadIdx.x + NT * k;
+        if (H == 1 || i < G::TILES * 256) { wsA[i] = sA[k]; wsB[i] = sB[k]; wsD[i] = sD[k]; }
       }
     }
   }
   if (a.pro) {
     __syncthreads();
-    bwd_node_prologue_finish<DE>(a, pro_ws, qd, b, l_begin, wg, proR);
+    bwd_node_prologue_finish<DE, H == 2>(a, pro_ws, qd, b, l_begin, wgp, proR);
   }
   if constexpr (MM != 0) {
     uint16_t* A16 = reinterpret_cast<uint16_t*>(wsA);
@@ -416,7 +428,7 @@
       hi = (uint16_t)h;
       lo = (uint16_t)(pk_bf16(v - __uint_as_float(h << 16), 0.f) & 0xFFFFu);
     };
-    for (int idx = threadIdx.x; idx < NS * 512; idx += 256) {
+    for (int idx = threadIdx.x; idx < NS * 512; idx += NT) {
       const int i = idx & 7, ln = (idx >> 3) & 63, s_ = idx >> 9, pp = ln & 15, qq = ln >> 4, t = 2 * s_ + (i >> 2);
       const int c = 16 * t + 4 * qq + (i & 3);
       const bool in = t < G::TILES && c < DE;
@@ -427,7 +439,7 @@
       parts((in && (pp & 2) == 0) ? a.Wr[hd * DE + c] : 0.f, hi, lo);
       B16[((s_ * 2 + 0) * 64 + ln) * 8 + i] = hi; B16[((s_ * 2 + 1) * 64 + ln) * 8 + i] = lo;
     }
-    for (int idx = threadIdx.x; idx < G::TILES * 256; idx += 256) {
+    for (int idx = threadIdx.x; idx < G::TILES * 256; idx += NT) {
       const int u = idx & 3, ln = (idx >> 2) & 63, t = idx >> 8, pp = ln & 15, qq = ln >> 4;
       uint16_t hi, lo;
       parts(a.pw[(16 * t + pp) * 16 + 4 * qq + u], hi, lo);
@@ -444,13 +456,15 @@
   float ssum[4] = {0.f, 0.f, 0.f, 0.f};
   __syncthreads();
 
-  for (int mt = mt_first; have && mt <= mt_last; mt += mt_step) {
+  const int mt_stop = H == 2 ? wave + 4 * ((ntile + 3) >> 2) : 0;
+  for (int mt = mt_first; H == 2 ? mt < mt_stop : (have && mt <= mt_last); mt += mt_step) {
+    const bool active = H == 1 || mt < ntile;
     const int r0 = (balance && mt == mt_first) ? r0_first : 0;
-    const int r1 = (balance && mt == mt_last) ? t1 - mt * nl : nl;
+    const int r1 = (balance && mt == mt_last) ? t1 - mt * nl : (active ? nl : 0);
     const int m0 = mt * 16, m = m0 + p;
     const int kv = RAG ? min(16, N - m0) : 16;
     const bool kvalid = RAG ? (p < kv) : true;
-    if (mt != mt_first) V5_TILE_START(mt, r0);
+    if (mt != mt_first && active) V5_TILE_START(mt, r0);
     float dKa[16], dVa[16];
 #pragma unroll
     for (int i = 0; i < 16; ++i) { dKa[i] = 0.f; dVa[i] = 0.f; }
@@ -695,6 +709,25 @@
         }
       }
     }
+    if constexpr (H == 2) {
+      float* park = sm + wave * 2048 + lane;
+      __syncthreads();
+      if (half == 1 && active) {
+#pragma unroll
+        for (int i = 0; i < 16; ++i) { park[i * 64] = dKa[i]; park[(16 + i) * 64] = dVa[i]; }
+      }
+      __syncthreads();
+      if (half == 0 && active) {
+#pragma unroll
+        for (int i = 0; i < 16; ++i) { dKa[i] += park[i * 64]; dVa[i] += park[(16 + i) * 64]; }
+#pragma unroll
+        for (int i = 0; i < 4; ++i) {
+          ko[i] = make_float4(dKa[4*i], dKa[4*i+1], dKa[4*i+2], dKa[4*i+3]);
+          vo[i] = make_float4(dVa[4*i], dVa[4*i+1], dVa[4*i+2], dVa[4*i+3]);
+        }
+      }
+      if (mt + 4 < mt_stop) __syncthreads();
+    } else
     if (kvalid) {
 #pragma unroll
       for (int i = 0; i < 4; ++i) {
@@ -711,7 +744,7 @@
 #pragma unroll
   for (int r = 0; r < 4; ++r) ssum[r] = row_sum16(ssum[r]);
   __syncthreads();
-  float* ep = sm + wave * G::EP;
+  float* ep = sm + wvw * G::EP;
 #pragma unroll
   for (int t = 0; t < G::TILES; ++t)
 #pragma unroll
@@ -725,8 +758,11 @@
   }
   __syncthreads();
   float* out = a.epart + (size_t)wg * G::EP;
-  for (int i = threadIdx.x; i < G::EP; i += 256)
-    out[i] = (sm[i] + sm[G::EP + i]) + (sm[2 * G::EP + i] + sm[3 * G::EP + i]);
+  for (int i = threadIdx.x; i < G::EP; i += NT) {
+    const float s03 = (sm[i] + sm[G::EP + i]) + (sm[2 * G::EP + i] + sm[3 * G::EP + i]);
+    if constexpr (H == 2) out[i] = s03 + ((sm[4 * G::EP + i] + sm[5 * G::EP + i]) + (sm[6 * G::EP + i] + sm[7 * G::EP + i]));
+    else out[i] = s03;
+  }
 }
 
 template <int DE, bool BF, int R>
diff --git a/egt_amd/csrc/egt_block_dev.h b/egt_amd/csrc/egt_block_dev.h
--- a/egt_amd/csrc/egt_block_dev.h
+++ b/egt_amd/csrc/egt_block_dev.h
@@ -267,7 +267,7 @@
 
 #define BWD_PRO_COMMON()                                                                                   \
   constexpr int LD = 68, LD3 = 196;                                                                        \
-  const int t = threadIdx.x, lane = t & 63, wave = __builtin_amdgcn_readfirstlane(t >> 6);                        \
+  const int t = H2 ? (int)(threadIdx.x & 255) : (int)threadIdx.x, lane = t & 63, wave = __builtin_amdgcn_readfirstlane(t >> 6); \
   const int p = lane & 15, q = lane >> 4, N = a.N;                                                         \
   const size_t row0 = (size_t)b * N + l_begin;                                                             \
   const int lnrow = 4 * wave + q;                \
@@ -277,7 +277,7 @@
   const int Dh = D64 ? 64 : a.Dh;                                                                          \
   (void)LD; (void)LD3; (void)lnrow; (void)p; (void)q; (void)rc; (void)Dh
 
-template <int DE, bool D64>
+template <int DE, bool D64, bool H2 = false>
 __device__ __forceinline__ void bwd_prologue_load_wo_va(const BlockArgs& a, int b, int l_begin, BwdProRegs& R) {
   BWD_PRO_COMMON();
   const bool iok = D64 || 16 * wave + p < Dh;
@@ -287,7 +287,7 @@
 #pragma unroll
   for (int r = 0; r < 4; ++r) R.va[r] = iok ? a.v_att[rc(4 * q + r) * Dh + 16 * wave + p] : 0.f;
 }
-template <int DE, bool D64>
+template <int DE, bool D64, bool H2 = false>
 __device__ __forceinline__ void bwd_prologue_load_main(const BlockArgs& a, int b, int l_begin, BwdProRegs& R) {
   BWD_PRO_COMMON();
     const float4 z4 = make_float4(0.f, 0.f, 0.f, 0.f);
@@ -336,7 +336,7 @@
       R.wq[s] = reinterpret_cast<const float4*>(a.up_wfrag + WFRAG_BWQ)[(wave * 12 + s) * 64 + lane];
 }
 
-template <int DE, bool D64>
+template <int DE, bool D64, bool H2 = false>
 __device__ __forceinline__ void bwd_prologue_compute(const BlockArgs& a, float* ws, float* qd, int b, int l_begin, int wg, BwdProRegs& R) {
   float* dqs = ws;
   float* xs = dqs + 16 * 196;
@@ -442,7 +442,7 @@
     *reinterpret_cast<float4*>(dhs + (t >> 4) * LD + (t & 15) * 4) =
         make_float4(ok ? dv4.x : 0.f, ok ? dv4.y : 0.f, ok ? dv4.z : 0.f, ok ? dv4.w : 0.f);
   }
-  bwd_prologue_load_wo_va<DE, D64>(a, b, l_begin, R);
+  bwd_prologue_load_wo_va<DE, D64, H2>(a, b, l_begin, R);
   __syncthreads();
   {
     v4f acc = {0.f, 0.f, 0.f, 0.f};
@@ -486,16 +486,16 @@
   if (a.pro == 2) bwd_prologue_load_main<DE, D64>(a, b, l_begin, R);
   bwd_prologue_compute<DE, D64>(a, ws, qd, b, l_begin, wg, R);
 }
-template <int DE>
+template <int DE, bool H2 = false>
 __device__ __forceinline__ void bwd_node_prologue_load(const BlockArgs& a, BwdProRegs& R, int b, int l_begin) {
   if (a.pro != 2) return;
-  if (a.Dh == 64) bwd_prologue_load_main<DE, true>(a, b, l_begin, R);
-  else bwd_prologue_load_main<DE, false>(a, b, l_begin, R);
-}
-template <int DE>
+  if (a.Dh == 64) bwd_prologue_load_main<DE, true, H2>(a, b, l_begin, R);
+  else bwd_prologue_load_main<DE, false, H2>(a, b, l_begin, R);
+}
+template <int DE, bool H2 = false>
 __device__ __forceinline__ void bwd_node_prologue_finish(const BlockArgs& a, float* ws, float* qd, int b, int l_begin, int wg, BwdProRegs& R) {
-  if (a.Dh == 64) bwd_prologue_compute<DE, true>(a, ws, qd, b, l_begin, wg, R);
-  else bwd_prologue_compute<DE, false>(a, ws, qd, b, l_begin, wg, R);
+  if (a.Dh == 64) bwd_prologue_compute<DE, true, H2>(a, ws, qd, b, l_begin, wg, R);
+  else bwd_prologue_compute<DE, false, H2>(a, ws, qd, b, l_begin, wg, R);
 }
 __device__ __forceinline__ void bwd_node_prologue_idle(const BlockArgs& a) {
   if (a.pro == 2) { __syncthreads(); __syncthreads(); }
diff --git a/include/egt_amd.h b/include/egt_amd.h
--- a/include/egt_amd.h
+++ b/include/egt_amd.h
@@ -163,6 +163,7 @@
 int egt_block_supported(const egt_block_desc* desc);
 const char* egt_block_bwd_kernel(const egt_block_desc* desc);
 const char* egt_block_launch_form(const egt_block_desc* desc);
+int egt_block_bwd_rows(const egt_block_desc* desc);
 size_t egt_block_saved_bytes(const egt_block_desc* desc);
 size_t egt_block_workspace_bytes(const egt_block_desc* desc);
 
```

Result: no change. 79380 graphs/s, median of 4 (-0.1%).
